# qasimyu/scssim

Hardware: AMD Instinct MI355X
Metric: paired-end read pairs/s (whole genreads job: MALBAC amplification + read allocation + read generation + FASTQ files, PE150 30x) (higher is better)
Workload: dtype u8/u32 (integer draws, byte sequences; fp64 only in the GC-weight draw and the allocation sums)

## Files before the change

scssim_amd/csrc/scs_device.h:

```cpp
#pragma once
#include <stdint.h>
#include <hip/hip_runtime.h>
#include "scs_common.h"
#include "scs_simuvars.h"

namespace scs {

struct DevFrags {
    const uint64_t* goff;
    const uint32_t* len;
    const int8_t*   strand;
    const uint32_t* primers;
    uint32_t n;
    uint64_t gidx_base;
    const uint8_t* has_n;
};

struct DevAmps {
    uint32_t* parent;
    uint32_t* sl;
    uint16_t* gc;
    uint16_t* primers;
    uint64_t* uid;
    uint64_t* errs;
};

struct DevGenomeIdx { const unsigned long long* gc_bits; const unsigned long long* n_bits; const uint64_t* gc_pref; const uint64_t* n_pref;
                      const ulonglong2* gc_pair; };

struct DevErrPool { uint32_t* data; uint32_t* head; uint32_t cap; };

struct View { int64_t base; int32_t dir; uint32_t comp; };

struct DevTables {
    int L, bins;
    uint32_t t_insert, t_delete, t_indel, t_ber;
    const uint32_t* gap_t; uint32_t t_kind;
    const uint32_t* subs1; const uint32_t* subs2;
    const uint32_t* qual;
    const uint4* ring1; const uint4* ring2;
    const uint4* ring1u; const uint4* ring2u;
    const uint32_t* qual_alias; int qual_k;
    const uint32_t* ins_t; int n_ins;
    const uint32_t* del_t; int n_del;
    const uint32_t* isize_t; int n_isize; int isize_min;
    const double* subs1_d; const double* subs2_d; const double* qual_d;
    const double* ins_d; const double* del_d; const double* isize_d;
    const double* gc_means; double gc_std;
};

struct AmplifyParams {
    RngKey key;
    uint32_t pass;
    uint32_t amp_min, amp_max;
    uint32_t t_ber;
};

struct PoissonParams {
    RngKey key; uint32_t call; double gamma;
    uint64_t total_primers;
    const uint64_t* totals;
    uint64_t nf, frag_len; const unsigned long long* dev;
    const unsigned long long* total_primers_dev;
};
enum { DS_HOLES = 20 };
enum { DS_SEMI_LEN = 4, DS_SEMIS_N = 5, DS_REPORTED_LEN = 6, DS_G_SEMIS_N = 8, DS_G_SEMI_LEN = 9, DS_G_PRIMERS = 10, DS_G_TOTALS = 11, DS_G_NF = 13, DS_G_FRAG_LEN = 14,
       DS_MIN_STOCK = 15 };
enum { SHARD_TAIL_WORDS = 16 };
struct AllocState { double total; unsigned long long sum_rn, sum_quota; };

#define ALLOC_CHUNK 1000u
enum { ALLOC_SLOTS = 40 };
struct AllocRange { uint32_t q0, c0, local0; };
struct AllocBChunk { uint32_t c, n, owner; };
struct AllocGSeg { unsigned long long go; uint32_t lo, n, owner, slot; };
struct AllocMySeg { unsigned long long go; uint32_t lo, n, order, pad; };
struct AllocPlan {
    unsigned long long total;
    uint32_t rank, n_interior, n_boundary, n_ranges, n_gseg;
    const AllocRange* rng; const AllocBChunk* bchunk; const AllocGSeg* gseg;
    AllocMySeg my_seg[ALLOC_SLOTS];
};
struct SegMap { uint32_t n; uint32_t lo[ALLOC_SLOTS], cnt[ALLOC_SLOTS]; unsigned long long go[ALLOC_SLOTS]; };

enum DevFlag : uint32_t { FLAG_ERRCAP = 1, FLAG_ERRPOOL = 2, FLAG_READSLOT = 4, FLAG_INTERNAL = 8, FLAG_KEYSPACE = 16, FLAG_TRUTH = 32, FLAG_DEPTH = 64, FLAG_AMP = 128, FLAG_SITE = 256, FLAG_SUPPORT = 512, FLAG_LIFT = 1024 };

struct PairRec {
    uint32_t amp, att, pos, isz;
    int64_t  base; uint32_t flags;
    int32_t  k1;
    uint64_t e1, e2, uid;
};

void launch_attach_frags(hipStream_t s, const uint8_t* g, DevFrags fr, const uint32_t* slot_off, uint32_t* slots,
                         uint32_t* slot_tmpl, uint32_t* valid, const unsigned long long* primer_cut, uint32_t* primer_delta,
                         unsigned long long* len_part, AmplifyParams p, uint32_t t_first, uint32_t t_end, int undo, const unsigned long long* t_from);
void launch_frag_len_sum(hipStream_t s, const unsigned long long* len_part, uint32_t nf, unsigned long long* len_sum);
void launch_poisson(hipStream_t s, DevFrags fr, DevAmps semis, uint32_t n_semis, PoissonParams p, uint32_t* budget_f, uint32_t* budget_s,
                    unsigned long long* sums, unsigned long long* part, uint32_t* flags);
void launch_alloc_bpack(hipStream_t s, const double* w, const AllocPlan& pl, double* send);
void launch_alloc_bgather(hipStream_t s, const double* w, const AllocPlan& pl, const double* gathered, double* brow, int* bmap);
void launch_alloc_chunk_sum(hipStream_t s, const double* w, const double* brow, const AllocPlan& pl, double* part);
void launch_tree_sum(hipStream_t s, const double* part, uint32_t nch, double* scratch, double* total);
void launch_alloc_norm(hipStream_t s, double* w, double* brow, const int* bmap, const AllocPlan& pl, const double* total, unsigned long long reads,
                       uint32_t* rn, double* tp, uint32_t* crn, unsigned long long* sum_rn);
void launch_alloc_quota(hipStream_t s, const double* tp, uint32_t nch, unsigned long long reads, const unsigned long long* sum_rn, unsigned long long* sum_quota,
                        uint32_t* quota, double* probs, double* scratch, RngKey key);
void launch_alloc_sample(hipStream_t s, const double* w, const double* brow, const int* bmap, const AllocPlan& pl, const double* tp, const uint32_t* quota, RngKey key, uint32_t* rn);
void launch_alloc_odd_scan(hipStream_t s, const uint32_t* rn, uint32_t ac, uint32_t* odd_before, void* temp, size_t temp_bytes);
void launch_alloc_odd_counts(hipStream_t s, const uint32_t* odd_before, const AllocPlan& pl, unsigned long long* table);
void launch_alloc_parity(hipStream_t s, uint32_t* rn, const uint32_t* odd_before, uint32_t ac, const AllocPlan& pl, const unsigned long long* table);
void launch_attach_semis(hipStream_t s, const uint8_t* g, DevFrags fr, DevAmps semis, uint32_t n_semis, DevErrPool spool,
                         const uint32_t* slot_off, uint32_t* slots, uint32_t* slot_tmpl, uint32_t* valid,
                         const unsigned long long* primer_cut, uint32_t* primer_delta, AmplifyParams p, uint32_t t_first, uint32_t t_end, int undo, const unsigned long long* t_from);
uint32_t attach_dense_waves(uint32_t n_slots);
void launch_attach_plan(hipStream_t s, const uint32_t* slot_off, uint32_t nt, uint32_t n_slots, uint32_t* item_tmpl, uint32_t* wave_first, uint32_t* valid);
void launch_attach_dense(hipStream_t s, const uint8_t* g, DevFrags fr, DevAmps semis, DevErrPool spool, const uint32_t* slot_off, uint32_t* slots, const uint32_t* item_tmpl,
                         const uint32_t* wave_first, uint32_t n_slots, uint32_t* valid, const unsigned long long* primer_cut, uint32_t* primer_delta, AmplifyParams p, int undo,
                         const unsigned long long* t_from);
void launch_stock_check(hipStream_t s, const int64_t* cnt, const uint32_t* taken, unsigned long long* cut, bool from_frag, unsigned long long* info);
void launch_stock_list(hipStream_t s, const int64_t* cnt, const uint32_t* taken, uint32_t* eidx, uint32_t* etype, uint32_t* estart, unsigned long long* info);
void launch_stock_collect(hipStream_t s, const uint8_t* g, DevFrags fr, DevAmps semis, DevErrPool spool, bool from_frag, const uint32_t* slot_off, const uint32_t* slots,
                          const uint32_t* valid, const uint32_t* eidx, unsigned long long* list, unsigned long long* info, uint32_t t_first, uint32_t t_end);
size_t stock_sort_temp_bytes(size_t n);
void launch_stock_sort(hipStream_t s, const unsigned long long* in, unsigned long long* out, size_t n, void* temp, size_t temp_bytes);
void launch_stock_pick(hipStream_t s, const int64_t* cnt, const uint32_t* etype, const uint32_t* estart, uint32_t ne, const unsigned long long* sorted, unsigned long long* cut,
                       bool from_frag, unsigned long long* info);
void launch_stock_apply(hipStream_t s, int64_t* cnt, uint32_t* gdelta, uint32_t* delta, unsigned long long* cut, uint32_t* flags);
void launch_errs_frags(hipStream_t s, const uint8_t* g, DevGenomeIdx gx, DevFrags fr, uint32_t n_slots, const uint32_t* slot_off, const uint32_t* slots,
                       const uint32_t* slot_tmpl, const uint32_t* valid_off, DevAmps out, uint32_t out_base, DevErrPool pool, uint32_t* flags,
                       const unsigned long long* binom, AmplifyParams p, int64_t* primer_cnt, uint32_t* primer_delta, unsigned long long* primer_cut, unsigned long long* sums,
                       unsigned long long* semis_n);
void launch_errs_semis(hipStream_t s, const uint8_t* g, DevGenomeIdx gx, DevFrags fr, DevAmps semis, uint32_t n_semis, DevErrPool spool, uint32_t n_slots,
                       const uint32_t* slot_off, const uint32_t* slots, const uint32_t* slot_tmpl, const uint32_t* valid_off,
                       DevAmps out, uint32_t out_base, DevErrPool pool, uint32_t* flags, const unsigned long long* binom, AmplifyParams p,
                       int64_t* primer_cnt, uint32_t* primer_delta, unsigned long long* primer_cut, unsigned long long* sums);
void launch_encode_bases(hipStream_t s, uint8_t* g, uint64_t n);
void launch_fa_gather_regular(hipStream_t s, const uint8_t* raw, uint8_t* dst, uint64_t n, uint32_t col0, uint32_t lb, uint32_t lw, uint32_t* ragged);
void launch_frag_has_n(hipStream_t s, const uint64_t* goff, const uint32_t* len, uint32_t nf, DevGenomeIdx gx, uint8_t* has_n);
size_t fasta_chunk_temp_bytes(uint32_t n);
void launch_fasta_chunk(hipStream_t s, const uint8_t* raw, uint32_t n, unsigned long long chunk_off, unsigned long long* st, uint8_t* kind, uint32_t* keep, uint32_t* pos,
                        uint8_t* out, unsigned long long* hdr, uint32_t hdr_cap, void* temp, size_t temp_bytes);
void launch_sv_build(hipStream_t s, const uint8_t* ref, const uint8_t* lit, const SvPiece* pieces, uint32_t np, const SvSubst* subs, uint32_t nsub, uint8_t* out, uint64_t total);
void launch_genome_bits(hipStream_t s, const uint8_t* g, uint64_t n, uint64_t nwords, unsigned long long* gc_bits, unsigned long long* n_bits,
                        uint32_t* gc_cnt, uint32_t* n_cnt, uint64_t* gc_pref, uint64_t* n_pref, void* temp, size_t temp_bytes, uint32_t* g2, ulonglong2* gc_pair);
void launch_amplify_init(hipStream_t s, int64_t* primer_cnt, unsigned long long* primer_cut, int64_t copies, uint32_t* primer_delta, uint32_t* primer_gdelta, uint32_t* flags, unsigned long long* sums,
                         unsigned long long nf_all, unsigned long long frag_len_all, unsigned long long total_primers, uint32_t* pool_head_a, uint32_t* pool_head_b);
void launch_primer_update(hipStream_t s, int64_t* primer_cnt, uint32_t* primer_delta, unsigned long long* primer_cut, unsigned long long* dsums, uint32_t* flags);
void launch_weights(hipStream_t s, DevAmps fulls, uint32_t n, DevTables tb, RngKey key, uint32_t frag_size, double* w);
void launch_plan_pairs(hipStream_t s, DevFrags fr, DevAmps semis, DevAmps fulls, uint32_t first, uint32_t n_fulls, uint32_t pair_lo, uint32_t pair_hi, const uint32_t* read_numbers,
                       const uint32_t* pair_off, SegMap gmap, DevTables tb, RngKey key, int paired, PairRec* pairs, unsigned long long* holes);
void launch_batch_bounds(hipStream_t s, const uint32_t* pair_off, uint32_t ac, unsigned long long batch, uint32_t nb, uint32_t* bounds);
void launch_parity_pair_offsets(hipStream_t s, uint32_t* rn, uint32_t ac, uint32_t* pair_cnt_off, void* temp, size_t temp_bytes);
void launch_pair_offsets(hipStream_t s, const uint32_t* rn, uint32_t ac, int paired, uint32_t* pair_cnt_off, void* temp, size_t temp_bytes);
struct ReadsSide {
    hipStream_t st[2] = {nullptr, nullptr}; hipEvent_t fork = nullptr, join[2] = {nullptr, nullptr}; void release();
    ReadsSide() = default; ReadsSide(const ReadsSide&) = delete; ReadsSide& operator=(const ReadsSide&) = delete; ~ReadsSide() { release(); }
};
size_t reads_lds_bytes(const DevTables& tb, bool uni = false);
struct BatchSet { uint32_t* ev_hdr; uint4* ev_dat; uint32_t* sizes[2]; uint64_t* off[2]; uint32_t *d1f[2], *d1p[2], *slist[2], *clist[2], *dlist[2]; };
struct BatchCounts { uint64_t bytes[2]; uint32_t n_general[2], n_one_event[2]; };
struct ReadsJob { const uint8_t* g; const uint32_t* g2; DevErrPool spool, fpool; DevTables tb; RngKey key; int paired; uint32_t slot; uint32_t* flags; ReadsSide* side; uint32_t amp_index_base = 0; };
void launch_reads(hipStream_t s, const ReadsJob& J, const PairRec* pairs, uint32_t np, const BatchSet& B, const BatchCounts& n, char* const out[2]);
void launch_read_lists(hipStream_t s, uint32_t np, int paired, const BatchSet& B, void* temp, size_t temp_bytes);
void phase_clock_report();
void launch_indels(hipStream_t s, const ReadsJob& J, const PairRec* pairs, uint32_t np, const BatchSet& B);
void launch_predict_windows(hipStream_t s, const uint8_t* windows, uint32_t n_reads, const uint64_t* uids, const uint32_t* atts,
                            const uint8_t* is_read1, DevTables tb, const DevTables* d_tb, RngKey key, uint32_t slot, char* slot_b, char* slot_q,
                            uint32_t* lens, uint32_t* flags);
void launch_text_checksum(hipStream_t s, const char* text, uint64_t nbytes, unsigned long long* out);
void launch_philox(hipStream_t s, const uint32_t* ctr, uint32_t n, RngKey key, uint32_t* out);
void launch_detlog(hipStream_t s, const double* x, uint32_t n, double* out);

#define MAIL_SEQ_SLOT 31
void launch_mail(hipStream_t s, const void* const* srcs, const int* widths, const int* dsts, int n, unsigned clear, unsigned long long* mail, unsigned long long seq);
void launch_shard_tail(hipStream_t s, uint32_t* primer_gdelta, const unsigned long long* dsums, const uint32_t* new_semis, int with_budgets);
void launch_primer_update_sharded(hipStream_t s, int64_t* primer_cnt, uint32_t* primer_gdelta, uint32_t* primer_delta, unsigned long long* primer_cut, unsigned long long* dsums, uint32_t* flags, int with_budgets);

hipError_t take_launch_error();

size_t scan_temp_bytes(size_t n);
size_t parity_scan_temp_bytes(size_t n);
void exclusive_scan_u32(hipStream_t s, const uint32_t* in, uint32_t* out, size_t n, void* temp, size_t temp_bytes);
void exclusive_scan_u32_pair(hipStream_t s, const uint32_t* in0, uint32_t* out0, size_t n0, const uint32_t* in1, uint32_t* out1, size_t n1, void* temp, size_t temp_bytes);
#define OFF_BITS 40
#define OFF_MASK ((1ull << OFF_BITS) - 1ull)
void exclusive_scan_sizes(hipStream_t s, const uint32_t* in, uint64_t* out, size_t n, void* temp, size_t temp_bytes);
void exclusive_scan_u32_to_u64(hipStream_t s, const uint32_t* in, uint64_t* out, size_t n, void* temp, size_t temp_bytes);

struct PlaceArgs {
    const PairRec* pairs; uint32_t np; int paired;
    const uint32_t* ev_hdr; const uint4* ev_dat;
    DevTables tb; RngKey key; uint32_t slot; uint32_t* flags;
};
struct TruthArgs : PlaceArgs {
    const uint64_t* off1; const uint64_t* off2; const char* fq1; const char* fq2;
    const uint8_t* g;
    const uint64_t* rec_off; const uint32_t* name_off; const char* names; uint32_t n_rec;
};
void launch_truth_size(hipStream_t s, const TruthArgs& a, uint32_t* sizes);
uint32_t truth_pairs_per_block(uint64_t fq_bytes, uint32_t np);
void launch_truth_emit(hipStream_t s, const TruthArgs& a, const uint64_t* offs, uint32_t pairs_per_block, char* out);
void launch_truth_bam_size(hipStream_t s, const TruthArgs& a, uint32_t* sizes);
uint32_t truth_bam_pairs_per_block(uint64_t fq_bytes, uint32_t np);
void launch_truth_bam_emit(hipStream_t s, const TruthArgs& a, const uint64_t* offs, uint32_t pairs_per_block, uint32_t lds, char* out);

struct DepthArgs : PlaceArgs {
    const uint64_t* rec_off; const uint64_t* bin_off; uint32_t n_rec;
    uint32_t bin_width, slots;
    unsigned long long* reads; unsigned long long* bases;
};
void launch_depth(hipStream_t s, const DepthArgs& a);

struct LiftSeg;
struct LiftArgs : PlaceArgs {
    const uint64_t* rec_off; uint32_t n_rec;
    const LiftSeg* segs; uint32_t n_seg;
    const uint64_t* ref_len; const uint64_t* ref_bin_off; uint32_t n_ref;
    uint32_t bin_width, slots; uint64_t n_bins;
    unsigned long long* reads; unsigned long long* bases;
};
void launch_depth_lift(hipStream_t s, const LiftArgs& a);
void launch_lift_copies(hipStream_t s, const LiftSeg* segs, uint32_t n_seg, const uint64_t* ref_len, const uint64_t* ref_bin_off, uint32_t n_ref, uint32_t bin_width,
                        uint64_t n_bins, unsigned long long* copies, uint32_t* flags);
void launch_lift_points(hipStream_t s, const LiftSeg* segs, uint32_t n_seg, const uint64_t* rec_off, uint32_t n_rec, const uint32_t* rec, const uint64_t* pos, uint64_t n,
                        uint32_t* ref_rec, uint64_t* ref_pos, uint32_t* kind, uint32_t* bad);

struct AmpArgs {
    DevFrags fr; DevAmps semis, fulls; const uint32_t* spool; const uint32_t* fpool;
    const uint8_t* g; const uint32_t* read_numbers;
    const uint64_t* rec_off; const uint32_t* name_off; const char* names; uint32_t n_rec;
    uint32_t first, n; uint32_t* flags;
};
#define AMP_LDS 16384u
void launch_amp_place(hipStream_t s, const AmpArgs& a, uint32_t* rec, uint64_t* start, uint32_t* len, int8_t* strand, uint32_t* n_edits);
void launch_amp_size(hipStream_t s, const AmpArgs& a, uint32_t* sizes);
void launch_amp_emit(hipStream_t s, const AmpArgs& a, const uint64_t* offs, uint32_t lds, char* out);

struct SiteRec;
struct SiteArgs {
    const uint64_t* keys; const uint32_t* reads; uint64_t n;
    const uint64_t* starts; const uint64_t* ps_start; const uint64_t* ends; const uint64_t* ps_end; uint64_t m;
    const uint8_t* g; const uint64_t* rec_off; const uint32_t* name_off; const char* names; uint32_t n_rec, min_reads; uint32_t* flags;
};
#define SITE_LDS 16384u
#define SITE_LDS_SLABS 1024u
void launch_site_count(hipStream_t s, const AmpArgs& a, uint64_t slab, uint32_t n_slabs, unsigned long long* cnt);
void launch_site_fill(hipStream_t s, const AmpArgs& a, uint64_t x0, uint64_t x1, unsigned long long* cur, uint64_t cap_e, uint64_t cap_a,
                      uint64_t* keys, uint32_t* kreads, uint64_t* starts, uint64_t* ends, uint32_t* areads);
void launch_site_check(hipStream_t s, const unsigned long long* cur, uint64_t n_e, uint64_t n_a, uint32_t* flags);
size_t site_sort_temp_bytes(size_t n);
void launch_site_sort(hipStream_t s, const uint64_t* keys_in, uint64_t* keys_out, const uint32_t* vals_in, uint32_t* vals_out, size_t n, unsigned end_bit, void* temp, size_t temp_bytes);
void launch_site_reduce(hipStream_t s, const SiteArgs& t, SiteRec* recs, uint32_t* sizes, uint32_t* keep);
void launch_site_emit(hipStream_t s, const SiteArgs& t, const SiteRec* recs, const uint64_t* offs, uint32_t lds, char* out, const uint32_t* site_pos = nullptr, const uint32_t* counts = nullptr);
void launch_site_compact(hipStream_t s, const SiteRec* recs, const uint32_t* keep, const uint32_t* pos, uint64_t n, SiteRec* out);

#define SUPPORT_MAX_POS ((1u << 29) - 1u)
#define SUPPORT_LDS_SLOTS 1024u
struct SupportArgs : PlaceArgs {
    const uint64_t* off1; const uint64_t* off2; const char* fq1; const char* fq2;
    const uint64_t* rec_off; uint32_t n_rec;
    const uint64_t* sp_pos; uint64_t n_pos;
    uint32_t* counts; uint32_t slots;
};
void launch_support(hipStream_t s, const SupportArgs& a);
void launch_support_heads(hipStream_t s, const SiteRec* sites, uint64_t n, const uint64_t* rec_off, uint32_t n_rec, uint32_t* head, uint32_t* flags);
void launch_support_scatter(hipStream_t s, const SiteRec* sites, uint64_t n, const uint64_t* rec_off, const uint32_t* head, const uint32_t* e, uint64_t* pos, uint32_t* site_pos);
void launch_support_size(hipStream_t s, const SiteArgs& t, const SiteRec* sites, const uint32_t* site_pos, const uint32_t* counts, uint32_t* sizes);

}
```

scssim_amd/csrc/scs_k_allocate.hip:

```cpp
#include <utility>
#include <type_traits>
#include "scs_device.h"
#include "scs_seams.h"

#include <algorithm>
#include <cstdlib>
#include <cstring>
#include <rocprim/rocprim.hpp>
#include "scs_kernels_common.h"

namespace scs {

struct GcDraw { double y, r2; bool in; };
__device__ __forceinline__ GcDraw gc_attempt(uint32_t wx, uint32_t wy) {
    const double x = 2.0 * (((double)wx + 0.5) / 4294967296.0) - 1.0;
    const double y = 2.0 * (((double)wy + 0.5) / 4294967296.0) - 1.0;
    const double r2 = x * x + y * y;
    return GcDraw{y, r2, !(r2 > 1.0 || r2 == 0.0)};
}
__device__ __forceinline__ double gc_value(double mean, double sd, double y, double r2) {
    const double mult = __dsqrt_rn(-2.0 * det_log(r2) / r2);
    return mean + sd * (y * mult);
}
constexpr int WEIGHTS_BLOCK = 1024;
__global__ __launch_bounds__(WEIGHTS_BLOCK) void k_weights(DevAmps fulls, uint32_t n, DevTables tb, RngKey key, uint32_t frag_size, double* __restrict__ w) {
    __shared__ uint32_t s_retry[WEIGHTS_BLOCK];
    __shared__ uint32_t s_n;
    if (threadIdx.x == 0) s_n = 0;
    __syncthreads();
    const uint32_t i = blockIdx.x * blockDim.x + threadIdx.x;
    const double scale = (double)(frag_size * frag_size), sd = tb.gc_std;
    if (i < n) {
        const uint32_t len = sl_len(fulls.sl[i]);
        const uint32_t gcp = 100u * fulls.gc[i] / len;
        if (gcp > 100) w[i] = 0.0 * (double)len / scale;
        else {
            const U4 d = draw4(key, ST_WEIGHT, 0, fulls.uid[i], 0);
            const GcDraw a0 = gc_attempt(d.w[0], d.w[1]), a1 = gc_attempt(d.w[2], d.w[3]);
            const bool any = a0.in || a1.in;
            double v = -1.0;
            if (any) v = gc_value(tb.gc_means[gcp], sd, a0.in ? a0.y : a1.y, a0.in ? a0.r2 : a1.r2);
            if (v < 0) s_retry[atomicAdd(&s_n, 1u)] = threadIdx.x | ((any && a0.in ? 1u : 2u) << 16);
            else w[i] = v * (double)len / scale;
        }
    }
    __syncthreads();
    const uint32_t nr = s_n;
    for (uint32_t k = threadIdx.x; k < nr; k += blockDim.x) {
        const uint32_t e = s_retry[k], j = blockIdx.x * blockDim.x + (e & 0xFFFFu);
        const uint32_t len = sl_len(fulls.sl[j]);
        const double mean = tb.gc_means[100u * fulls.gc[j] / len];
        const uint64_t uid = fulls.uid[j];
        uint32_t a = e >> 16;
        U4 d = draw4(key, ST_WEIGHT, 0, uid, a >> 1);
        double v;
        for (;; ++a) {
            if ((a & 1u) == 0 && a != (e >> 16)) d = draw4(key, ST_WEIGHT, 0, uid, a >> 1);
            const GcDraw t = (a & 1u) ? gc_attempt(d.w[2], d.w[3]) : gc_attempt(d.w[0], d.w[1]);
            if (!t.in) continue;
            v = gc_value(mean, sd, t.y, t.r2);
            if (v >= 0) break;
        }
        w[j] = v * (double)len / scale;
    }
}

__device__ __forceinline__ double shfl_xor_f64(double v, int d) {
    const long long b = __double_as_longlong(v);
    const int lo = __shfl_xor((int)b, d), hi = __shfl_xor((int)(b >> 32), d);
    return __longlong_as_double(((long long)hi << 32) | (unsigned int)lo);
}
__device__ __forceinline__ double shfl_up_f64(double v, int d) {
    const long long b = __double_as_longlong(v);
    const int lo = __shfl_up((int)b, d), hi = __shfl_up((int)(b >> 32), d);
    return __longlong_as_double(((long long)hi << 32) | (unsigned int)lo);
}
__device__ __forceinline__ double shfl_f64(double v, int src) {
    const long long b = __double_as_longlong(v);
    const int lo = __shfl((int)b, src), hi = __shfl((int)(b >> 32), src);
    return __longlong_as_double(((long long)hi << 32) | (unsigned int)lo);
}
__device__ __forceinline__ double wave_butterfly_f64(double acc) {
#pragma unroll
    for (int d = 32; d >= 1; d >>= 1) acc = acc + shfl_xor_f64(acc, d);
    return acc;
}
struct ChunkRef { uint32_t c, n, local0; int brow; bool owner; };
__device__ __forceinline__ ChunkRef chunk_ref(const AllocPlan& pl, uint32_t q) {
    ChunkRef r;
    if (q < pl.n_interior) {
        uint32_t k = 0;
        while (k + 1 < pl.n_ranges && q >= pl.rng[k + 1].q0) ++k;
        const AllocRange& g = pl.rng[k];
        r.c = g.c0 + (q - g.q0); r.local0 = g.local0 + (q - g.q0) * ALLOC_CHUNK; r.brow = -1; r.owner = true;
        const unsigned long long b = (unsigned long long)r.c * ALLOC_CHUNK;
        r.n = (uint32_t)min((unsigned long long)ALLOC_CHUNK, pl.total - b);
    } else {
        const uint32_t bi = q - pl.n_interior;
        r.c = pl.bchunk[bi].c; r.n = pl.bchunk[bi].n; r.local0 = 0; r.brow = (int)bi; r.owner = pl.bchunk[bi].owner != 0;
    }
    return r;
}
__global__ void __launch_bounds__(256) k_alloc_bpack(const double* __restrict__ w, AllocPlan pl, double* __restrict__ send) {
    const uint32_t slot = blockIdx.x / 2, half = blockIdx.x & 1u;
    const uint32_t n = pl.my_seg[slot].n, lo = pl.my_seg[slot].lo, m = min(n, ALLOC_CHUNK);
    for (uint32_t i = threadIdx.x; i < ALLOC_CHUNK; i += blockDim.x)
        send[((size_t)slot * 2 + half) * ALLOC_CHUNK + i] = i < m ? w[lo + (half ? n - m + i : i)] : 0.0;
}
__global__ void __launch_bounds__(256) k_alloc_bgather(const double* __restrict__ w, AllocPlan pl, const double* __restrict__ gathered,
                                                       double* __restrict__ brow, int* __restrict__ bmap) {
    const uint32_t bi = blockIdx.x;
    const unsigned long long g0 = (unsigned long long)pl.bchunk[bi].c * ALLOC_CHUNK;
    for (uint32_t e = threadIdx.x; e < ALLOC_CHUNK; e += blockDim.x) {
        double v = 0; int mp = -1;
        if (e < pl.bchunk[bi].n) {
            const unsigned long long gi = g0 + e;
            uint32_t lo = 0, hi = pl.n_gseg;
            while (hi - lo > 1) { const uint32_t mid = (lo + hi) >> 1; if (pl.gseg[mid].go <= gi) lo = mid; else hi = mid; }
            const AllocGSeg sg = pl.gseg[lo];
            const uint32_t j = (uint32_t)(gi - sg.go);
            if (sg.owner == pl.rank) { mp = (int)(sg.lo + j); v = w[sg.lo + j]; }
            else {
                const double* src = gathered + ((size_t)sg.owner * ALLOC_SLOTS + sg.slot) * 2 * ALLOC_CHUNK;
                v = j < ALLOC_CHUNK ? src[j] : src[ALLOC_CHUNK + (j - (sg.n - ALLOC_CHUNK))];
            }
        }
        brow[(size_t)bi * ALLOC_CHUNK + e] = v; bmap[(size_t)bi * ALLOC_CHUNK + e] = mp;
    }
}
__global__ void __launch_bounds__(256) k_alloc_chunk_sum(const double* __restrict__ w, const double* __restrict__ brow, AllocPlan pl,
                                                         double* __restrict__ part) {
    const uint32_t q = blockIdx.x * 4 + (threadIdx.x >> 6), lane = threadIdx.x & 63;
    if (q >= pl.n_interior + pl.n_boundary) return;
    const ChunkRef r = chunk_ref(pl, q);
    const double* __restrict__ v = r.brow < 0 ? w + r.local0 : brow + (size_t)r.brow * ALLOC_CHUNK;
    double acc = 0;
    for (uint32_t i = lane; i < r.n; i += WAVE) acc += v[i];
    acc = wave_butterfly_f64(acc);
    if (lane == 0 && r.owner) part[r.c] = acc;
}
__global__ void __launch_bounds__(256) k_tree1000(const double* __restrict__ in, uint32_t n, double* __restrict__ out) {
    const uint32_t gq = blockIdx.x * 4 + (threadIdx.x >> 6), lane = threadIdx.x & 63;
    const uint32_t b = gq * ALLOC_CHUNK;
    if (b >= n) return;
    const uint32_t m = min(ALLOC_CHUNK, n - b);
    double acc = 0;
    for (uint32_t i = lane; i < m; i += WAVE) acc += in[b + i];
    acc = wave_butterfly_f64(acc);
    if (lane == 0) out[gq] = acc;
}
__global__ void __launch_bounds__(256) k_alloc_norm(double* __restrict__ w, double* __restrict__ brow, const int* __restrict__ bmap, AllocPlan pl,
                                                    const double* __restrict__ total, unsigned long long reads, uint32_t* __restrict__ rn,
                                                    double* __restrict__ tp, uint32_t* __restrict__ crn) {
    const uint32_t q = blockIdx.x * 4 + (threadIdx.x >> 6), lane = threadIdx.x & 63;
    if (q >= pl.n_interior + pl.n_boundary) return;
    const ChunkRef r = chunk_ref(pl, q);
    double* __restrict__ v = r.brow < 0 ? w + r.local0 : brow + (size_t)r.brow * ALLOC_CHUNK;
    const int* __restrict__ mp = r.brow < 0 ? nullptr : bmap + (size_t)r.brow * ALLOC_CHUNK;
    const double den = 2.2204e-16 + *total;
    double acc = 0; uint32_t cs = 0;
    for (uint32_t i = lane; i < r.n; i += WAVE) {
        const double p = v[i] / den;
        v[i] = p; acc += p;
        const uint32_t c = (uint32_t)(p * (double)(long long)reads);
        if (mp) { const int li = mp[i]; if (li >= 0) { rn[li] = c; cs += c; } }
        else { rn[r.local0 + i] = c; cs += c; }
    }
    acc = wave_butterfly_f64(acc);
    cs = wave_sum(cs);
    if (lane == 0) { if (r.owner) tp[r.c] = acc; crn[q] = cs; }
}
__global__ void __launch_bounds__(1024) k_sum_u32(const uint32_t* __restrict__ v, uint32_t n, unsigned long long* __restrict__ dst, int add) {
    __shared__ unsigned long long s_p[16];
    unsigned long long acc = 0;
    for (uint32_t i = threadIdx.x; i < n; i += blockDim.x) acc += v[i];
    acc = wave_sum_u64(acc);
    if ((threadIdx.x & 63) == 0) s_p[threadIdx.x >> 6] = acc;
    __syncthreads();
    if (threadIdx.x == 0) { unsigned long long t = 0; for (int k = 0; k < 16; ++k) t += s_p[k]; *dst = add ? *dst + t : t; }
}
__global__ void __launch_bounds__(256) k_alloc_quota(const double* __restrict__ tp, uint32_t nch, unsigned long long reads, const unsigned long long* __restrict__ sum_rn,
                                                     uint32_t* __restrict__ quota) {
    const uint32_t c = blockIdx.x * blockDim.x + threadIdx.x;
    if (c >= nch) return;
    const unsigned long long nres = reads - *sum_rn;
    quota[c] = (uint32_t)(tp[c] * (double)nres);
}
__global__ void __launch_bounds__(64) k_scan1000(const double* __restrict__ in, uint32_t n, double* __restrict__ out, double* __restrict__ last) {
    const uint32_t g = blockIdx.x, b = g * ALLOC_CHUNK, m = min(ALLOC_CHUNK, n - b), lane = threadIdx.x;
    double carry = 0;
    for (uint32_t r = 0; r < m; r += WAVE) {
        double s = r + lane < m ? in[b + r + lane] : 0.0;
#pragma unroll
        for (int d = 1; d < WAVE; d <<= 1) { const double t = shfl_up_f64(s, d); if ((int)lane >= d) s = s + t; }
        if (r + lane < m) out[b + r + lane] = carry + s;
        carry = carry + shfl_f64(s, 63);
    }
    if (lane == 0 && last) last[g] = carry;
}
__global__ void __launch_bounds__(256) k_scan_fix(double* __restrict__ out, uint32_t n, const double* __restrict__ pre) {
    const uint32_t i = blockIdx.x * blockDim.x + threadIdx.x;
    if (i >= n || i < ALLOC_CHUNK) return;
    out[i] = pre[i / ALLOC_CHUNK - 1] + out[i];
}
__device__ __forceinline__ uint32_t first_le(const double* __restrict__ cdf, uint32_t n, double r) {
    uint32_t lo = 0, hi = n;
    while (lo < hi) { const uint32_t mid = (lo + hi) >> 1; if (r <= cdf[mid]) hi = mid; else lo = mid + 1; }
    return lo < n ? lo : n - 1;
}
__global__ void k_alloc_top_draws(const double* __restrict__ probs, uint32_t nch, unsigned long long reads, const unsigned long long* __restrict__ sum_rn,
                                  const unsigned long long* __restrict__ sum_quota, RngKey key, uint32_t* __restrict__ quota) {
    const uint32_t t = blockIdx.x * blockDim.x + threadIdx.x;
    const unsigned long long n = reads - *sum_rn - *sum_quota;
    if (t >= n) return;
    const U4 d = draw4(key, ST_ALLOC_TOP, 0, 0, t);
    const double r = 2.2204e-16 + (1 - 2.2204e-16) * ((double)d.w[0] / 4294967296.0);
    atomicAdd(&quota[first_le(probs, nch, r)], 1u);
}
__global__ void __launch_bounds__(256) k_alloc_sample(const double* __restrict__ w, const double* __restrict__ brow, const int* __restrict__ bmap, AllocPlan pl,
                                                      const double* __restrict__ tp, const uint32_t* __restrict__ quota, RngKey key, uint32_t* __restrict__ rn) {
    constexpr int ROUNDS = (ALLOC_CHUNK + WAVE - 1) / WAVE, WAVES = 4, MINE = ROUNDS / WAVES;
    static_assert(ROUNDS % WAVES == 0, "rounds of scan1000 divide among the waves");
    __shared__ double s_cdf[ALLOC_CHUNK];
    __shared__ uint32_t s_cnt[ALLOC_CHUNK];
    __shared__ double s_tot[ROUNDS];
    const uint32_t q = blockIdx.x, tid = threadIdx.x, lane = tid & 63u, wv = tid >> 6;
    const ChunkRef r = chunk_ref(pl, q);
    const uint32_t nq = quota[r.c];
    if (nq == 0) return;
    const double* __restrict__ v = r.brow < 0 ? w + r.local0 : brow + (size_t)r.brow * ALLOC_CHUNK;
    const double t = tp[r.c];
    double pv[MINE];
#pragma unroll
    for (int m = 0; m < MINE; ++m) { const uint32_t i = (uint32_t)((wv + WAVES * m) * WAVE) + lane; pv[m] = i < r.n ? v[i] : 0.0; }
#pragma unroll
    for (int m = 0; m < MINE; ++m) {
        const uint32_t k = wv + WAVES * m, i = k * WAVE + lane;
        double s = i < r.n ? pv[m] / t : 0.0;
#pragma unroll
        for (int d = 1; d < WAVE; d <<= 1) { const double u = shfl_up_f64(s, d); if ((int)lane >= d) s = s + u; }
        pv[m] = s;
        if (lane == 63) s_tot[k] = s;
    }
    __syncthreads();
#pragma unroll
    for (int m = 0; m < MINE; ++m) {
        const uint32_t k = wv + WAVES * m, i = k * WAVE + lane;
        double carry = 0;
        for (uint32_t z = 0; z < k; ++z) carry = carry + s_tot[z];
        if (i < r.n) { s_cdf[i] = carry + pv[m]; s_cnt[i] = 0; }
    }
    __syncthreads();
    for (uint32_t j = tid; 4u * j < nq; j += blockDim.x) {
        const U4 d = draw4(key, ST_ALLOC_CHUNK, 0, r.c, j);
        double x[4]; uint32_t lo[4], hi[4];
#pragma unroll
        for (int i = 0; i < 4; ++i) { x[i] = 2.2204e-16 + (1 - 2.2204e-16) * ((double)d.w[i] / 4294967296.0); lo[i] = 0; hi[i] = r.n; }
        for (uint32_t span = r.n; span; span >>= 1) {
#pragma unroll
            for (int i = 0; i < 4; ++i)
                if (lo[i] < hi[i]) { const uint32_t mid = (lo[i] + hi[i]) >> 1; if (x[i] <= s_cdf[mid]) hi[i] = mid; else lo[i] = mid + 1; }
        }
#pragma unroll
        for (int i = 0; i < 4; ++i) if (4u * j + (uint32_t)i < nq) atomicAdd(&s_cnt[lo[i] < r.n ? lo[i] : r.n - 1], 1u);
    }
    __syncthreads();
    for (uint32_t i = tid; i < r.n; i += blockDim.x) {
        const uint32_t c = s_cnt[i];
        if (!c) continue;
        if (r.brow < 0) rn[r.local0 + i] += c;
        else { const int li = bmap[(size_t)r.brow * ALLOC_CHUNK + i]; if (li >= 0) rn[li] += c; }
    }
}
__global__ void k_alloc_odd_counts(const uint32_t* __restrict__ odd_before, AllocPlan pl, unsigned long long* __restrict__ table) {
    const uint32_t slot = threadIdx.x;
    if (slot >= ALLOC_SLOTS) return;
    const uint32_t n = pl.my_seg[slot].n, lo = pl.my_seg[slot].lo;
    table[(size_t)pl.my_seg[slot].order] = n ? odd_before[lo + n] - odd_before[lo] : 0u;
}
__global__ void __launch_bounds__(256) k_alloc_parity(uint32_t* __restrict__ rn, const uint32_t* __restrict__ odd_before, uint32_t ac, AllocPlan pl,
                                                      const unsigned long long* __restrict__ table) {
    __shared__ unsigned long long s_base[ALLOC_SLOTS];
    if (threadIdx.x < ALLOC_SLOTS) {
        unsigned long long b = 0;
        if (table) { const uint32_t ord = pl.my_seg[threadIdx.x].order; for (uint32_t k = 0; k < ord; ++k) b += table[k]; }
        s_base[threadIdx.x] = b;
    }
    __syncthreads();
    const uint32_t i = blockIdx.x * blockDim.x + threadIdx.x;
    if (i >= ac) return;
    const uint32_t v = rn[i];
    if (!(v & 1u)) return;
    unsigned long long j = odd_before[i];
    if (table) {
        uint32_t k = 0;
        while (k + 1 < ALLOC_SLOTS && (pl.my_seg[k].n == 0 || i >= pl.my_seg[k].lo + pl.my_seg[k].n)) ++k;
        j = s_base[k] + (odd_before[i] - odd_before[pl.my_seg[k].lo]);
    }
    rn[i] = (j & 1ull) ? v - 1u : v + 1u;
}

struct OddBit { __host__ __device__ uint32_t operator()(uint32_t v) const { return v & 1u; } };
struct HalfUp { __host__ __device__ uint32_t operator()(uint32_t v) const { return (v + 1u) >> 1; } };

void launch_alloc_bpack(hipStream_t s, const double* w, const AllocPlan& pl, double* send) {
    hipLaunchKernelGGL(k_alloc_bpack, dim3(2 * ALLOC_SLOTS), dim3(256), 0, s, w, pl, send);
}
void launch_alloc_bgather(hipStream_t s, const double* w, const AllocPlan& pl, const double* gathered, double* brow, int* bmap) {
    if (pl.n_boundary) hipLaunchKernelGGL(k_alloc_bgather, dim3(pl.n_boundary), dim3(256), 0, s, w, pl, gathered, brow, bmap);
}
void launch_alloc_chunk_sum(hipStream_t s, const double* w, const double* brow, const AllocPlan& pl, double* part) {
    const uint32_t nq = pl.n_interior + pl.n_boundary;
    if (nq) hipLaunchKernelGGL(k_alloc_chunk_sum, dim3(cdiv(nq, 4)), dim3(256), 0, s, w, brow, pl, part);
}
void launch_tree_sum(hipStream_t s, const double* part, uint32_t nch, double* scratch, double* total) {
    if (nch == 0) { (void)hipMemsetAsync(total, 0, 8, s); return; }
    if (nch == 1) { (void)hipMemcpyAsync(total, part, 8, hipMemcpyDeviceToDevice, s); return; }
    const double* cur = part; uint32_t n = nch; double* nxt = scratch;
    while (n > 1) {
        const uint32_t ng = cdiv(n, ALLOC_CHUNK);
        double* dst = ng == 1 ? total : nxt;
        hipLaunchKernelGGL(k_tree1000, dim3(cdiv(ng, 4)), dim3(256), 0, s, cur, n, dst);
        cur = dst; nxt += ng; n = ng;
    }
}
void launch_alloc_norm(hipStream_t s, double* w, double* brow, const int* bmap, const AllocPlan& pl, const double* total, unsigned long long reads,
                       uint32_t* rn, double* tp, uint32_t* crn, unsigned long long* sum_rn) {
    const uint32_t nq = pl.n_interior + pl.n_boundary;
    if (nq) hipLaunchKernelGGL(k_alloc_norm, dim3(cdiv(nq, 4)), dim3(256), 0, s, w, brow, bmap, pl, total, reads, rn, tp, crn);
    hipLaunchKernelGGL(k_sum_u32, dim3(1), dim3(1024), 0, s, crn, nq, sum_rn, 0);
}
static void scan_all_dev(hipStream_t s, const double* in, uint32_t n, double* out, double* scratch) {
    const uint32_t ng = cdiv(n, ALLOC_CHUNK);
    double* last = scratch; double* pre = scratch + ng;
    hipLaunchKernelGGL(k_scan1000, dim3(ng), dim3(64), 0, s, in, n, out, ng > 1 ? last : (double*)nullptr);
    if (ng == 1) return;
    scan_all_dev(s, last, ng, pre, scratch + 2 * (size_t)ng);
    hipLaunchKernelGGL(k_scan_fix, dim3(cdiv(n, 256)), dim3(256), 0, s, out, n, pre);
}
void launch_alloc_quota(hipStream_t s, const double* tp, uint32_t nch, unsigned long long reads, const unsigned long long* sum_rn, unsigned long long* sum_quota,
                        uint32_t* quota, double* probs, double* scratch, RngKey key) {
    if (nch == 0) return;
    hipLaunchKernelGGL(k_alloc_quota, dim3(cdiv(nch, 256)), dim3(256), 0, s, tp, nch, reads, sum_rn, quota);
    hipLaunchKernelGGL(k_sum_u32, dim3(1), dim3(1024), 0, s, quota, nch, sum_quota, 0);
    scan_all_dev(s, tp, nch, probs, scratch);
    hipLaunchKernelGGL(k_alloc_top_draws, dim3(cdiv((uint64_t)nch + 1024, 256)), dim3(256), 0, s, probs, nch, reads, sum_rn, sum_quota, key, quota);
}
void launch_alloc_sample(hipStream_t s, const double* w, const double* brow, const int* bmap, const AllocPlan& pl, const double* tp, const uint32_t* quota, RngKey key, uint32_t* rn) {
    const uint32_t nq = pl.n_interior + pl.n_boundary;
    if (nq) hipLaunchKernelGGL(k_alloc_sample, dim3(nq), dim3(256), 0, s, w, brow, bmap, pl, tp, quota, key, rn);
}
void launch_alloc_odd_scan(hipStream_t s, const uint32_t* rn, uint32_t ac, uint32_t* odd_before, void* temp, size_t temp_bytes) {
    (void)rocprim::exclusive_scan(temp, temp_bytes, rocprim::make_transform_iterator(rn, OddBit()), odd_before, 0u, (size_t)ac + 1, rocprim::plus<uint32_t>(), s);
}
void launch_alloc_odd_counts(hipStream_t s, const uint32_t* odd_before, const AllocPlan& pl, unsigned long long* table) {
    hipLaunchKernelGGL(k_alloc_odd_counts, dim3(1), dim3(64), 0, s, odd_before, pl, table);
}
void launch_alloc_parity(hipStream_t s, uint32_t* rn, const uint32_t* odd_before, uint32_t ac, const AllocPlan& pl, const unsigned long long* table) {
    if (ac) hipLaunchKernelGGL(k_alloc_parity, dim3(cdiv(ac, 256)), dim3(256), 0, s, rn, odd_before, ac, pl, table);
}
void launch_weights(hipStream_t s, DevAmps fulls, uint32_t n, DevTables tb, RngKey key, uint32_t frag_size, double* w) {
    if (n == 0) return;
    hipLaunchKernelGGL(k_weights, dim3(cdiv(n, (uint32_t)WEIGHTS_BLOCK)), dim3(WEIGHTS_BLOCK), 0, s, fulls, n, tb, key, frag_size, w);
}
using ScanCfg = rocprim::scan_config<256, 16, rocprim::block_load_method::block_load_transpose, rocprim::block_store_method::block_store_transpose, rocprim::block_scan_algorithm::using_warp_scan>;
struct PackOddHalf { __host__ __device__ uint64_t operator()(uint32_t v) const { return ((uint64_t)(v & 1u) << 32) | (uint64_t)(v >> 1); } };
struct ParityOut {
    struct Ref {
        uint32_t* rn; uint32_t* pair_off; size_t ac, i;
        __device__ const Ref& operator=(uint64_t sum) const {
            const uint32_t odd = (uint32_t)(sum >> 32);
            pair_off[i] = (uint32_t)sum + ((odd + 1u) >> 1);
            if (i < ac) { const uint32_t v = rn[i]; if (v & 1u) rn[i] = (odd & 1u) ? v - 1u : v + 1u; }
            return *this;
        }
    };
    using iterator_category = std::random_access_iterator_tag; using value_type = uint64_t; using difference_type = std::ptrdiff_t;
    using pointer = void; using reference = Ref;
    uint32_t* rn; uint32_t* pair_off; size_t ac, at;
    __host__ __device__ Ref operator[](difference_type k) const { return Ref{rn, pair_off, ac, at + (size_t)k}; }
    __host__ __device__ Ref operator*() const { return Ref{rn, pair_off, ac, at}; }
    __host__ __device__ ParityOut operator+(difference_type k) const { return ParityOut{rn, pair_off, ac, at + (size_t)k}; }
    __host__ __device__ ParityOut operator-(difference_type k) const { return ParityOut{rn, pair_off, ac, at - (size_t)k}; }
    __host__ __device__ ParityOut& operator+=(difference_type k) { at += (size_t)k; return *this; }
    __host__ __device__ ParityOut& operator++() { ++at; return *this; }
    __host__ __device__ difference_type operator-(const ParityOut& o) const { return (difference_type)at - (difference_type)o.at; }
};
size_t parity_scan_temp_bytes(size_t n) {
    size_t c3 = 0;
    (void)rocprim::exclusive_scan<ScanCfg>(nullptr, c3, rocprim::make_transform_iterator((const uint32_t*)nullptr, PackOddHalf()), ParityOut{nullptr, nullptr, 0, 0},
                                  (uint64_t)0, n + 1, rocprim::plus<uint64_t>());
    return c3;
}
void launch_parity_pair_offsets(hipStream_t s, uint32_t* rn, uint32_t ac, uint32_t* pair_cnt_off, void* temp, size_t temp_bytes) {
    (void)rocprim::exclusive_scan<ScanCfg>(temp, temp_bytes, rocprim::make_transform_iterator((const uint32_t*)rn, PackOddHalf()), ParityOut{rn, pair_cnt_off, (size_t)ac, 0},
                                  (uint64_t)0, (size_t)ac + 1, rocprim::plus<uint64_t>(), s);
}
void launch_pair_offsets(hipStream_t s, const uint32_t* rn, uint32_t ac, int paired, uint32_t* pair_cnt_off, void* temp, size_t temp_bytes) {
    if (paired) (void)rocprim::exclusive_scan(temp, temp_bytes, rocprim::make_transform_iterator(rn, HalfUp()), pair_cnt_off, 0u, (size_t)ac + 1, rocprim::plus<uint32_t>(), s);
    else (void)rocprim::exclusive_scan(temp, temp_bytes, rn, pair_cnt_off, 0u, (size_t)ac + 1, rocprim::plus<uint32_t>(), s);
}
}
```

scssim_amd/csrc/scs_reads.cpp:

```cpp
#include "scs_sink.h"
#include <cerrno>

namespace scs {
void do_allocate(scs_ctx* c, uint64_t reads) {
    if (!c->amplified) throw ScsError(SCS_EINVAL, "scs_allocate_reads: call scs_amplify first");
    hipStream_t s = c->stream;
    if (reads == 0) {
        uint64_t ref_len = 0;
        for (auto& r : c->recs) { size_t p = r.name.rfind('_'); ref_len += (uint64_t)atoi(r.name.c_str() + (p == std::string::npos ? 0 : p + 1)); }
        ref_len /= 2;
        reads = (uint64_t)(ref_len * c->cfg.coverage / (long)c->prof.read_length);
    }
    if (c->cfg.verbose) fprintf(stderr, "\nNumber of reads to generate: %llu\n", (unsigned long long)reads);
    c->reads_requested = reads; c->st.reads_requested = reads;
    const uint32_t ac = c->fulls.n;
    double t0 = now_s();
    c->weights.reserve(std::max<size_t>((size_t)ac * 8, 16), s);
    c->read_numbers.reserve(((size_t)ac + 1) * 4, s); c->pair_off.reserve(((size_t)ac + 1) * 4, s);
    launch_weights(s, c->fulls.view(), ac, c->dtb, c->key, (uint32_t)c->cfg.frag_size, c->weights.as<double>());
    double* d_w = c->weights.as<double>(); uint32_t* d_rn = c->read_numbers.as<uint32_t>();

    const int R = c->cfg.shard_count, me = c->cfg.shard_rank; const bool multi = c->sharded();
    std::vector<uint64_t> segc((size_t)R * ALLOC_SLOTS, 0);
    for (auto& sg : c->full_segs) { if (sg.c < 0 || sg.c >= 5 || sg.p < 0 || sg.p >= 8) throw ScsError(SCS_EINVAL, "allocation: segment out of range"); segc[(size_t)me * ALLOC_SLOTS + sg.c * 8 + (7 - sg.p)] += sg.count; }
    if (multi) c->reduce(segc.data(), segc.size());
    std::vector<AllocGSeg> gseg; std::vector<uint32_t> loff(R, 0); uint64_t total = 0;
    AllocPlan pl{}; pl.rank = (uint32_t)me;
    for (int sl = 0; sl < ALLOC_SLOTS; ++sl) for (int r = 0; r < R; ++r) {
        const uint64_t n = segc[(size_t)r * ALLOC_SLOTS + sl];
        if (r == me) pl.my_seg[sl] = AllocMySeg{total, loff[r], (uint32_t)n, (uint32_t)(sl * R + r), 0};
        if (!n) continue;
        gseg.push_back(AllocGSeg{total, loff[r], (uint32_t)n, (uint32_t)r, (uint32_t)sl});
        loff[r] += (uint32_t)n; total += n;
    }
    if (loff[me] != ac) throw ScsError(SCS_EINVAL, "sharded allocation: segment bookkeeping mismatch");
    if (total > 0xFFFFFFF0ull) throw ScsError(SCS_EOVERFLOW, "more than 2^32 amplicons in the whole job");
    const uint32_t nch = (uint32_t)((total + ALLOC_CHUNK - 1) / ALLOC_CHUNK);
    std::vector<AllocRange> rng; std::vector<AllocBChunk> bch; uint32_t nq = 0;
    {
        auto owner_of = [&](uint64_t gi) { size_t lo = 0, hi = gseg.size(); while (hi - lo > 1) { const size_t mid = (lo + hi) / 2; if (gseg[mid].go <= gi) lo = mid; else hi = mid; } return gseg[lo].owner; };
        auto add_boundary = [&](uint32_t ch) { for (auto& b : bch) if (b.c == ch) return; bch.push_back(AllocBChunk{ch, (uint32_t)std::min<uint64_t>(ALLOC_CHUNK, total - (uint64_t)ch * ALLOC_CHUNK), owner_of((uint64_t)ch * ALLOC_CHUNK) == (uint32_t)me ? 1u : 0u}); };
        for (size_t k = 0; k < gseg.size();) {
            if (gseg[k].owner != (uint32_t)me) { ++k; continue; }
            uint64_t go = gseg[k].go, n = gseg[k].n; const uint32_t lo = gseg[k].lo; size_t j = k + 1;
            while (j < gseg.size() && gseg[j].owner == (uint32_t)me && gseg[j].go == go + n) { n += gseg[j].n; ++j; }
            k = j;
            const uint64_t cA = (go + ALLOC_CHUNK - 1) / ALLOC_CHUNK, cB = go + n == total ? nch : (go + n) / ALLOC_CHUNK;
            if (cA < cB) { rng.push_back(AllocRange{nq, (uint32_t)cA, (uint32_t)(lo + (cA * ALLOC_CHUNK - go))}); nq += (uint32_t)(cB - cA); }
            if (cA >= cB) { for (uint64_t ch = go / ALLOC_CHUNK; ch <= (go + n - 1) / ALLOC_CHUNK; ++ch) add_boundary((uint32_t)ch); }
            else {
                if (go % ALLOC_CHUNK) add_boundary((uint32_t)(go / ALLOC_CHUNK));
                if (cB * ALLOC_CHUNK < go + n) add_boundary((uint32_t)cB);
            }
        }
    }
    pl.total = total; pl.n_interior = nq; pl.n_boundary = (uint32_t)bch.size(); pl.n_ranges = (uint32_t)rng.size(); pl.n_gseg = (uint32_t)gseg.size();
    const uint32_t nwork = pl.n_interior + pl.n_boundary;
    {
        const size_t o_b = rng.size() * sizeof(AllocRange), o_g = o_b + bch.size() * sizeof(AllocBChunk), bytes = o_g + gseg.size() * sizeof(AllocGSeg);
        std::vector<uint8_t> blob(std::max<size_t>(bytes, 16));
        if (!rng.empty()) memcpy(blob.data(), rng.data(), o_b);
        if (!bch.empty()) memcpy(blob.data() + o_b, bch.data(), o_g - o_b);
        if (!gseg.empty()) memcpy(blob.data() + o_g, gseg.data(), bytes - o_g);
        c->a_plan.reserve(blob.size(), s);
        HIP_OK(hipMemcpyAsync(c->a_plan.p, blob.data(), blob.size(), hipMemcpyHostToDevice, s)); HIP_OK(hipStreamSynchronize(s));
        pl.rng = (const AllocRange*)c->a_plan.p; pl.bchunk = (const AllocBChunk*)((char*)c->a_plan.p + o_b); pl.gseg = (const AllocGSeg*)((char*)c->a_plan.p + o_g);
    }
    for (int sl = 0; sl < ALLOC_SLOTS; ++sl) c->seg_lo[sl] = pl.my_seg[sl].lo;
    c->seg_lo[ALLOC_SLOTS] = ac;
    c->gmap = SegMap{};
    if (multi) { uint32_t k = 0; for (int sl = 0; sl < ALLOC_SLOTS; ++sl) if (pl.my_seg[sl].n) { c->gmap.lo[k] = pl.my_seg[sl].lo; c->gmap.cnt[k] = pl.my_seg[sl].n; c->gmap.go[k] = pl.my_seg[sl].go; ++k; } c->gmap.n = k; }

    const size_t tree_scratch = (size_t)nch / ALLOC_CHUNK * 3 + 4096;
    c->a_part.reserve(((size_t)nch + 2) * 8, s); c->a_tp.reserve(((size_t)nch + 2) * 8, s); c->a_probs.reserve(((size_t)nch + 2) * 8, s);
    c->a_quota.reserve(((size_t)nch + 2) * 4, s); c->a_crn.reserve(((size_t)nwork + 2) * 4, s); c->a_scratch.reserve(tree_scratch * 8, s);
    c->a_brow.reserve(std::max<size_t>((size_t)pl.n_boundary * ALLOC_CHUNK * 8, 16), s); c->a_bmap.reserve(std::max<size_t>((size_t)pl.n_boundary * ALLOC_CHUNK * 4, 16), s);
    c->odd_before.reserve(((size_t)ac + 1) * 4, s); c->scan_tmp.reserve(scan_temp_bytes(ac), s);
    AllocState* st = (AllocState*)((char*)c->dsums.p + 128);
    double* d_part = c->a_part.as<double>(); double* d_tp = c->a_tp.as<double>();
    unsigned long long* d_sum_rn = (unsigned long long*)(d_tp + nch);
    if (R > 1) {
        const size_t per = (size_t)ALLOC_SLOTS * 2 * ALLOC_CHUNK * 8;
        c->a_send.reserve(per, s); c->a_gath.reserve(per * R, s);
        launch_alloc_bpack(s, d_w, pl, c->a_send.as<double>());
        c->gather_dev(c->a_send.p, c->a_gath.p, per);
    }
    launch_alloc_bgather(s, d_w, pl, c->a_gath.as<double>(), c->a_brow.as<double>(), c->a_bmap.as<int>());
    if (multi) HIP_OK(hipMemsetAsync(d_part, 0, (size_t)nch * 8, s));
    launch_alloc_chunk_sum(s, d_w, c->a_brow.as<double>(), pl, d_part);
    if (multi) c->reduce_dev(d_part, nch, 8);
    launch_tree_sum(s, d_part, nch, c->a_scratch.as<double>(), &st->total);
    if (multi) HIP_OK(hipMemsetAsync(d_tp, 0, ((size_t)nch + 1) * 8, s));
    launch_alloc_norm(s, d_w, c->a_brow.as<double>(), c->a_bmap.as<int>(), pl, &st->total, reads, d_rn, d_tp, c->a_crn.as<uint32_t>(), d_sum_rn);
    if (multi) c->reduce_dev(d_tp, (uint64_t)nch + 1, 8);
    launch_alloc_quota(s, d_tp, nch, reads, d_sum_rn, &st->sum_quota, c->a_quota.as<uint32_t>(), c->a_probs.as<double>(), c->a_scratch.as<double>(), c->key);
    launch_alloc_sample(s, d_w, c->a_brow.as<double>(), c->a_bmap.as<int>(), pl, d_tp, c->a_quota.as<uint32_t>(), c->key, d_rn);
    if (c->cfg.paired && !multi) launch_parity_pair_offsets(s, d_rn, ac, c->pair_off.as<uint32_t>(), c->scan_tmp.p, c->scan_tmp.cap);
    else if (c->cfg.paired) {
        launch_alloc_odd_scan(s, d_rn, ac, c->odd_before.as<uint32_t>(), c->scan_tmp.p, c->scan_tmp.cap);
        unsigned long long* table = nullptr;
        if (multi) {
            c->a_odd.reserve((size_t)R * ALLOC_SLOTS * 8, s); table = c->a_odd.as<unsigned long long>();
            HIP_OK(hipMemsetAsync(table, 0, (size_t)R * ALLOC_SLOTS * 8, s));
            launch_alloc_odd_counts(s, c->odd_before.as<uint32_t>(), pl, table);
            c->reduce_dev(table, (uint64_t)R * ALLOC_SLOTS, 8);
        }
        launch_alloc_parity(s, d_rn, c->odd_before.as<uint32_t>(), ac, pl, table);
    }
    if (!c->cfg.paired || multi) launch_pair_offsets(s, d_rn, ac, c->cfg.paired != 0, c->pair_off.as<uint32_t>(), c->scan_tmp.p, c->scan_tmp.cap);
    { Mail m; m.add(ac ? (const void*)(c->pair_off.as<uint32_t>() + ac) : nullptr, 4, 0); mail_post(c, m, true); }
    mail_wait(c);
    c->n_pairs_planned = (uint32_t)c->h_rb[0];
    c->st.t_stage[3] = 0; c->st.t_stage[4] = now_s() - t0;
    c->allocated = true;
}

BatchPlan plan_batches(uint64_t P, uint32_t L, bool to_sink, int writers, int regions, int batch_shift) {
    BatchPlan pl; regions = to_sink ? std::max(1, regions) : 1;
    uint64_t sink_batch = 1ull << 19;
    if (to_sink && writers > 4) {
        const uint64_t per_part = P / (2ull * (uint64_t)regions);
        sink_batch = 1ull << 18; while (sink_batch < (1ull << 21) && sink_batch * 2 <= per_part) sink_batch <<= 1;
        const uint64_t per_pair = 4ull * L + 64ull;
        while (sink_batch > (1ull << 18) && ((uint64_t)writers + 2ull) * sink_batch * per_pair > (24ull << 30)) sink_batch >>= 1;
    }
    pl.batch = std::min<uint64_t>(std::max<uint64_t>(P, 1), batch_shift ? (1ull << batch_shift) : to_sink ? sink_batch : (1ull << 23));
    const uint32_t nbatch = pl.nbatch = (uint32_t)((P + pl.batch - 1) / pl.batch);
    const int n_writers = to_sink ? std::max(1, std::min(writers, regions)) : 1;
    pl.order.reserve(nbatch); pl.region_of.reserve(nbatch);
    for (int g0 = 0; g0 < regions; g0 += n_writers) {
        const int g1 = std::min(regions, g0 + n_writers);
        std::vector<uint32_t> next((size_t)(g1 - g0)), end((size_t)(g1 - g0)); size_t left = 0;
        for (int r = g0; r < g1; ++r) { next[(size_t)(r - g0)] = (uint32_t)((uint64_t)nbatch * r / regions); end[(size_t)(r - g0)] = (uint32_t)((uint64_t)nbatch * (r + 1) / regions); left += end[(size_t)(r - g0)] - next[(size_t)(r - g0)]; }
        while (left) for (int r = g0; r < g1; ++r) if (next[(size_t)(r - g0)] < end[(size_t)(r - g0)]) { pl.order.push_back(next[(size_t)(r - g0)]++); pl.region_of.push_back((uint32_t)r); --left; }
    }
    return pl;
}

namespace {
struct Ship { char* p[3]; uint64_t n[3]; int dsl; uint32_t region; };
struct Batch { uint64_t it, p0; uint32_t bidx, np; int k, dsl; const PairRec* pr; const BatchSet* B; BatchCounts n; char* out[2]; char* t_text; uint64_t t_n; };
struct SegAt { size_t seg; uint32_t b; uint64_t o[2]; };
struct FdGuard { int fd = -1; ~FdGuard() { if (fd >= 0) ::close(fd); } };
struct PipeGuard { SinkPipe* p; ~PipeGuard() { if (p) (void)p->finish(); } };

struct Yield {
    scs_ctx* const c; const OutTarget& tg;
    const hipStream_t s = c->stream; hipStream_t ps = s; const int paired = c->cfg.paired != 0; const uint64_t P = c->n_pairs_planned; const uint32_t L = (uint32_t)c->prof.read_length, slot = ((L + 64 + 63) / 64) * 64;
    const bool to_sink = !tg.device && tg.sink, truth = !c->truth_path.empty(), bam = truth && c->truth_bam, bgzf = to_sink && tg.bgzf, depth = c->depth_width != 0, depth_ref = c->dref_width != 0, support = c->support_on; const std::string tname = bam ? "truth BAM" : "truth SAM";
    BatchPlan plan; std::vector<uint32_t> bounds; BatchSet bs[2]; ReadsJob job;
    uint64_t tot[2] = {0, 0}, sunk[2] = {0, 0}, truth_sum = 0, bi = 0;
    bool d2h_rec[2] = {false, false}, free_rec[2] = {false, false}; Ship pending{}; bool have_pending = false;
    FdGuard truth_fd;
    PipeGuard guard{nullptr}; TruthArgs ta{}; DepthArgs da{}; LiftArgs la{}; SupportArgs sa{};
    std::vector<uint64_t> bpair, bb[2]; std::vector<SegAt> seg_at;
    void truth_open() {
        truth_fd.fd = ::open(c->truth_path.c_str(), O_WRONLY | O_CREAT | O_TRUNC | O_CLOEXEC, 0644);
        if (truth_fd.fd < 0) throw ScsError(SCS_EIO, tname + ": can not open " + c->truth_path + ": " + strerror(errno));
        std::string hd = "@HD\tVN:1.6\tSO:unsorted\n"; const uint32_t nr = (uint32_t)c->recs.size();
        std::vector<uint64_t> roff(nr + 1, 0); std::vector<uint32_t> noff(nr + 1, 0); std::string names;
        for (uint32_t r = 0; r < nr; ++r) {
            hd += "@SQ\tSN:" + c->recs[r].name + "\tLN:" + std::to_string(c->rec_len[r]) + "\n";
            roff[r] = c->rec_off[r]; roff[r + 1] = c->rec_off[r] + c->rec_len[r];
            names += c->recs[r].name; noff[r + 1] = (uint32_t)names.size();
        }
        hd += "@PG\tID:scssim\tPN:scssim\n";
        if (bam) {
            std::string bh = "BAM\1";
            auto le32 = [&](uint32_t v) { for (int k = 0; k < 4; ++k) bh.push_back((char)(v >> (8 * k))); };
            le32((uint32_t)hd.size()); bh += hd; le32(nr);
            for (uint32_t r = 0; r < nr; ++r) { le32((uint32_t)c->recs[r].name.size() + 1u); bh += c->recs[r].name; bh.push_back('\0'); le32((uint32_t)c->rec_len[r]); }
            std::vector<uint8_t> z; bgzf_compress_host((const uint8_t*)bh.data(), bh.size(), BGZF_LDS_OUT, z);
            hd.assign((const char*)z.data(), z.size());
        }
        if (!SinkPipe::write_all(truth_fd.fd, hd.data(), hd.size())) throw ScsError(SCS_EIO, tname + ": writing " + c->truth_path + " failed");
        truth_sum = hd.size();
        const size_t o_name = (size_t)(nr + 1) * 8, o_text = o_name + (size_t)(nr + 1) * 4; std::vector<uint8_t> blob(o_text + names.size() + 16, 0);
        memcpy(blob.data(), roff.data(), o_name); memcpy(blob.data() + o_name, noff.data(), (size_t)(nr + 1) * 4); memcpy(blob.data() + o_text, names.data(), names.size());
        upload(c->t_recs, blob, s);
        c->t_sizes.reserve((plan.batch + 1) * 4, s); c->t_offs.reserve((plan.batch + 1) * 8, s); c->t_scan.reserve(scan_temp_bytes(plan.batch), s);
        c->h_t.reserve(64, hipHostMallocDefault); c->ev_t.ensure(hipEventDisableTiming | hipEventBlockingSync);
        HIP_OK(hipStreamSynchronize(s));
        const uint8_t* tb = c->t_recs.as<uint8_t>();
        ta.g = c->genome.as<uint8_t>(); ta.rec_off = (const uint64_t*)tb; ta.name_off = (const uint32_t*)(tb + o_name); ta.names = (const char*)(tb + o_text); ta.n_rec = nr;
        ta.paired = paired; ta.tb = c->dtb; ta.key = c->key; ta.slot = slot; ta.flags = c->flags.as<uint32_t>();
    }
    void depth_open() {
        static const uint32_t slots = seam_env("SCS_TEST_DEPTH_SLOTS") ? (uint32_t)atoi(seam_env("SCS_TEST_DEPTH_SLOTS")) : DEPTH_LDS_SLOTS;
        const uint32_t nr = (uint32_t)c->recs.size(); std::vector<uint64_t> tab(2 * ((size_t)nr + 1), 0), boff;
        const uint64_t nb = c->depth_bins = depth_ctx_layout(c, &boff);
        for (uint32_t r = 0; r < nr; ++r) { tab[r] = c->rec_off[r]; tab[r + 1] = c->rec_off[r] + c->rec_len[r]; }
        std::copy(boff.begin(), boff.end(), tab.begin() + nr + 1);
        upload(c->dp_tab, tab, s);
        c->dp_cnt.reserve(std::max<size_t>((size_t)nb * 16, 16), s); HIP_OK(hipMemsetAsync(c->dp_cnt.p, 0, std::max<size_t>((size_t)nb * 16, 16), s));
        HIP_OK(hipStreamSynchronize(s));
        da.rec_off = c->dp_tab.as<uint64_t>(); da.bin_off = da.rec_off + nr + 1; da.n_rec = nr; da.bin_width = c->depth_width; da.slots = slots;
        da.reads = c->dp_cnt.as<unsigned long long>(); da.bases = da.reads + nb;
        da.paired = paired; da.tb = c->dtb; da.key = c->key; da.slot = slot; da.flags = c->flags.as<uint32_t>();
    }
    void depth_ref_open() {
        static const uint32_t slots = seam_env("SCS_TEST_LIFT_SLOTS") ? (uint32_t)atoi(seam_env("SCS_TEST_LIFT_SLOTS")) : DEPTH_LDS_SLOTS;
        scs::depth_ref_open(c);
        const uint32_t nr = (uint32_t)c->recs.size(), nf = (uint32_t)c->lift.ref_lens.size(); const uint64_t nb = c->dref_bins;
        la.rec_off = c->dr_tab.as<uint64_t>(); la.n_rec = nr; la.ref_len = la.rec_off + nr + 1; la.ref_bin_off = la.ref_len + nf; la.n_ref = nf;
        la.segs = c->d_lift.as<LiftSeg>(); la.n_seg = (uint32_t)c->lift.segs.size(); la.bin_width = c->dref_width; la.slots = slots; la.n_bins = nb;
        la.reads = c->dr_cnt.as<unsigned long long>(); la.bases = la.reads + nb + 1;
        la.paired = paired; la.tb = c->dtb; la.key = c->key; la.slot = slot; la.flags = c->flags.as<uint32_t>();
    }
    void support_open() {
        static const uint32_t slots = seam_env("SCS_TEST_SUPPORT_SLOTS") ? (uint32_t)atoi(seam_env("SCS_TEST_SUPPORT_SLOTS")) : SUPPORT_LDS_SLOTS;
        scs::support_open(c);
        sa.rec_off = c->sp_tab.as<uint64_t>(); sa.n_rec = (uint32_t)c->recs.size(); sa.sp_pos = c->sp_pos.as<uint64_t>(); sa.n_pos = c->sp_n_pos;
        sa.counts = c->sp_cnt.as<uint32_t>(); sa.slots = slots;
        sa.paired = paired; sa.tb = c->dtb; sa.key = c->key; sa.slot = slot; sa.flags = c->flags.as<uint32_t>();
    }
    void setup() {
        bounds.assign(plan.nbatch + 1, 0);
        if (P) {
            c->d_bounds.reserve(((size_t)plan.nbatch + 1) * 4, s);
            launch_batch_bounds(s, c->pair_off.as<uint32_t>(), c->fulls.n, plan.batch, plan.nbatch, c->d_bounds.as<uint32_t>());
            HIP_OK(hipMemcpyAsync(bounds.data(), c->d_bounds.p, ((size_t)plan.nbatch + 1) * 4, hipMemcpyDeviceToHost, s)); HIP_OK(hipStreamSynchronize(s));
        }
        if (truth) truth_open();
        if (depth) depth_open();
        if (depth_ref) depth_ref_open();
        if (support) support_open();
        if (to_sink) {
            if (!c->pipe) c->pipe.reset(new SinkPipe);
            c->copy_stream.ensure(hipStreamNonBlocking); for (int k = 0; k < 2; ++k) { c->ev_made[k].ensure(hipEventDisableTiming); c->ev_d2h[k].ensure(hipEventDisableTiming); }
            c->pipe->truth_fd = truth_fd.fd; c->pipe->start(tg.sink, paired != 0, c->cfg.device); guard.p = c->pipe.get();
        }
        if (bgzf || bam) { c->h_z.reserve(64, hipHostMallocDefault); memset(c->h_z, 0, 64); for (int k = 0; k < 2; ++k) c->ev_z[k].ensure(hipEventDisableTiming | hipEventBlockingSync); }
        if ((bgzf || bam) && !c->z_crc.p) {
            std::vector<uint32_t> tabs(512); bgzf_host_tables(tabs.data(), tabs.data() + 256); upload(c->z_crc, tabs, s); HIP_OK(hipStreamSynchronize(s));
        }
        const uint64_t batch = plan.batch, nreads_b = paired ? 2 * batch : batch;
        c->ev_hdr.reserve(2 * nreads_b * 4, s); c->ev_dat.reserve(2 * nreads_b * 16, s);
        for (int m = 0; m < 2; ++m) c->sizes[m].reserve(2 * (batch + 1) * 4, s);
        for (int m = 0; m < 2; ++m) c->off[m].reserve(2 * (batch + 1) * 8, s);
        c->scan_tmp.reserve(scan_temp_bytes(batch), s);
        c->rl_cls.reserve(2 * (batch + 1) * 2 * 4, s); c->rl_pos.reserve(2 * (batch + 1) * 2 * 4, s); c->rl_lists.reserve(2 * batch * 6 * 4, s);
        for (int k = 0; k < 2; ++k) {
            BatchSet& B = bs[k]; B.ev_hdr = c->ev_hdr.as<uint32_t>() + k * nreads_b; B.ev_dat = c->ev_dat.as<uint4>() + k * nreads_b;
            for (int m = 0; m < 2; ++m) {
                B.sizes[m] = c->sizes[m].as<uint32_t>() + k * (batch + 1); B.off[m] = c->off[m].as<uint64_t>() + k * (batch + 1);
                B.d1f[m] = c->rl_cls.as<uint32_t>() + (k * 2 + m) * (batch + 1); B.d1p[m] = c->rl_pos.as<uint32_t>() + (k * 2 + m) * (batch + 1);
                B.slist[m] = c->rl_lists.as<uint32_t>() + (k * 6 + m) * batch; B.clist[m] = B.slist[m] + 2 * batch; B.dlist[m] = B.slist[m] + 4 * batch;
            }
        }
        job = ReadsJob{c->genome.as<uint8_t>(), c->genome2.as<uint32_t>() + 16, c->semis.pool_view(), c->fulls.pool_view(), c->dtb, c->key, paired, slot, c->flags.as<uint32_t>(), &c->reads_side};
        static const bool serial_pre = seam_env("SCS_READS_SERIAL") != nullptr;
        if (!serial_pre) {
            c->pre_stream.ensure(hipStreamNonBlocking); c->ev_plan.ensure(hipEventDisableTiming); for (int k = 0; k < 2; ++k) { c->ev_pre[k].ensure(hipEventDisableTiming); c->ev_free[k].ensure(hipEventDisableTiming); }
            ps = c->pre_stream; HIP_OK(hipEventRecord(c->ev_plan, s)); HIP_OK(hipStreamWaitEvent(ps, c->ev_plan, 0));
        }
        bb[0].assign(plan.nbatch, 0); bb[1].assign(plan.nbatch, 0);
        if (!tg.seg_off1) return;
        std::vector<uint32_t> v(ALLOC_SLOTS + 1, 0);
        for (int k = 0; k <= ALLOC_SLOTS; ++k) HIP_OK(hipMemcpyAsync(&v[k], c->pair_off.as<uint32_t>() + c->seg_lo[k], 4, hipMemcpyDeviceToHost, s));
        HIP_OK(hipStreamSynchronize(s));
        bpair.assign(v.begin(), v.end()); tg.seg_off1->assign(ALLOC_SLOTS + 1, 0); if (tg.seg_off2) tg.seg_off2->assign(ALLOC_SLOTS + 1, 0);
    }
    void prepass(uint64_t it) {
        hipStream_t s = ps;
        const int k = (int)(it & 1); const BatchSet& B = bs[k]; const uint64_t batch = plan.batch, p0 = (uint64_t)plan.order[it] * batch;
        if (ps != c->stream && free_rec[k]) HIP_OK(hipStreamWaitEvent(ps, c->ev_free[k], 0));
        const uint32_t np = (uint32_t)std::min<uint64_t>(batch, P - p0);
        const PairRec* pr = c->pairs.as<PairRec>() + p0;
        const uint32_t b = (uint32_t)(p0 / batch), a_lo = bounds[b], a_hi = std::min<uint32_t>(c->fulls.n, bounds[b + 1] + 1u);
        launch_plan_pairs(s, c->frags_view(), c->semis.view(), c->fulls.view(), a_lo, a_hi - a_lo, (uint32_t)p0, (uint32_t)(p0 + np), c->read_numbers.as<uint32_t>(), c->pair_off.as<uint32_t>(),
                          c->gmap, c->dtb, c->key, paired, c->pairs.as<PairRec>(), c->dsums.as<unsigned long long>() + DS_HOLES);
        c->tm[TM_INDELS].begin(s);
        launch_indels(s, job, pr, np, B);
        c->tm[TM_INDELS].end(s); c->tm[TM_INDELS].add_units(np);
        for (int m = 0; m < (paired ? 2 : 1); ++m) exclusive_scan_sizes(s, B.sizes[m], B.off[m], np, c->scan_tmp.p, c->scan_tmp.cap);
        launch_read_lists(s, np, paired, B, c->scan_tmp.p, c->scan_tmp.cap);
        Mail m; m.add(B.off[0] + np, 8, 0); m.add(paired ? (const void*)(B.off[1] + np) : nullptr, 8, 1);
        m.add(B.d1p[0] + np, 4, 2); m.add(paired ? (const void*)(B.d1p[1] + np) : nullptr, 4, 3); mail_post(c, m, true, s);
        if (ps != c->stream) HIP_OK(hipEventRecord(c->ev_pre[k], ps));
    }
    Batch decode(uint64_t it) const {
        Batch b{}; b.it = it; b.k = (int)(it & 1); b.bidx = plan.order[it]; b.p0 = (uint64_t)b.bidx * plan.batch; b.np = (uint32_t)std::min<uint64_t>(plan.batch, P - b.p0);
        b.pr = c->pairs.as<PairRec>() + b.p0; b.B = &bs[b.k]; b.dsl = (int)(bi & 1);
        for (int m = 0; m < 2; ++m) { b.n.bytes[m] = c->h_rb[m] & OFF_MASK; b.n.n_general[m] = (uint32_t)(c->h_rb[m] >> OFF_BITS); b.n.n_one_event[m] = (uint32_t)c->h_rb[2 + m]; }
        if (seam_env("SCS_DEBUG_CLASSES")) fprintf(stderr, "[classes] batch of %u pairs: general %u / %u, one-event %u / %u\n", b.np, b.n.n_general[0], b.n.n_general[1], b.n.n_one_event[0], b.n.n_one_event[1]);
        return b;
    }
    void index_batch(const Batch& b) {
        for (int m = 0; m < 2; ++m) bb[m][b.bidx] = b.n.bytes[m];
        for (size_t j = (size_t)(std::lower_bound(bpair.begin(), bpair.end(), b.p0) - bpair.begin()); j < bpair.size() && bpair[j] < b.p0 + b.np; ++j) {
            uint64_t ov[2] = {0, 0}; const uint64_t idx = bpair[j] - b.p0;
            for (int m = 0; m < (paired ? 2 : 1); ++m) HIP_OK(hipMemcpyAsync(&ov[m], b.B->off[m] + idx, 8, hipMemcpyDeviceToHost, s));
            HIP_OK(hipStreamSynchronize(s)); seg_at.push_back(SegAt{j, b.bidx, {ov[0] & OFF_MASK, ov[1] & OFF_MASK}});
        }
    }
    void reserve_slot(DevBuf* d, int nb, const uint64_t* need, const uint64_t* room, int dsl, bool stream_wait) {
        bool grows = false; for (int i = 0; i < nb; ++i) grows |= need[i] > d[i].cap;
        if (d2h_rec[dsl] && grows) HIP_OK(hipEventSynchronize(c->ev_d2h[dsl]));
        else if (d2h_rec[dsl] && stream_wait) HIP_OK(hipStreamWaitEvent(s, c->ev_d2h[dsl], 0));
        for (int i = 0; i < nb; ++i) d[i].reserve(room[i], s);
    }
    void base_pass(Batch& b) {
        if (tg.device) {
            if (tot[0] + b.n.bytes[0] > tg.cap1 || tot[1] + b.n.bytes[1] > tg.cap2) throw ScsError(SCS_EOVERFLOW, "scs_yield_reads_device: output buffer too small");
            b.out[0] = tg.d1 + tot[0]; b.out[1] = tg.d2 ? tg.d2 + tot[1] : nullptr;
        } else {
            DevBuf* d = c->out[b.dsl];
            const uint64_t want[2] = {std::max<uint64_t>(b.n.bytes[0] + b.n.bytes[0] / 16, 16), std::max<uint64_t>(b.n.bytes[1] + b.n.bytes[1] / 16, 16)};
            reserve_slot(d, 2, want, want, b.dsl, true);
            b.out[0] = d[0].as<char>(); b.out[1] = d[1].as<char>();
        }
        c->tm[TM_READS].begin(s);
        launch_reads(s, job, b.pr, b.np, *b.B, b.n, b.out);
        c->tm[TM_READS].end(s); c->tm[TM_READS].add_units(b.np);
        if (c->want_cks && !tg.device) for (int m = 0; m < 2; ++m) launch_text_checksum(s, b.out[m], m && !paired ? 0 : b.n.bytes[m], c->d_cks.as<unsigned long long>() + 2 * (size_t)b.bidx + m);
    }
    char* bgzf_in_place(int lane, const char* text, uint64_t n, int dsl, const char* too_large) {
        if (bgzf_bound(n) > 0xFFFFFFF0ull) throw ScsError(SCS_EOVERFLOW, too_large);
        scs_ctx::BgzfLane& z = c->z[lane]; DevBuf& zo = z.out[dsl]; const uint32_t nblk = bgzf_blocks(n); const uint64_t zb = bgzf_bound(n);
        z.plan.reserve(std::max<size_t>((size_t)nblk * BGZF_PLAN_BYTES, 16), s); z.sizes.reserve(((size_t)nblk + 2) * 4, s); z.offs.reserve(((size_t)nblk + 2) * 4, s);
        reserve_slot(&zo, 1, &zb, &zb, dsl, false);
        launch_bgzf_plan(s, text, n, z.plan.as<uint8_t>(), z.sizes.as<uint32_t>());
        exclusive_scan_u32(s, z.sizes.as<uint32_t>(), z.offs.as<uint32_t>(), nblk, nullptr, 0);
        launch_bgzf_emit(s, text, n, z.plan.as<uint8_t>(), z.sizes.as<uint32_t>(), z.offs.as<uint32_t>(), c->z_crc.as<uint32_t>(), c->z_crc.as<uint32_t>() + 256, zo.as<char>(), 0);
        HIP_OK(hipMemcpyAsync(c->h_z + (dsl * 3 + lane), z.offs.as<uint32_t>() + nblk, 4, hipMemcpyDeviceToHost, s));
        return zo.as<char>();
    }
    void truth_batch(Batch& b) {
        static const uint32_t bam_lds = seam_env("SCS_TEST_TRUTH_LDS") ? (uint32_t)atoi(seam_env("SCS_TEST_TRUTH_LDS")) : 0u;
        const uint32_t np = b.np; const uint64_t fq_bytes = b.n.bytes[0] + b.n.bytes[1];
        ta.pairs = b.pr; ta.np = np; ta.ev_hdr = b.B->ev_hdr; ta.ev_dat = b.B->ev_dat; ta.off1 = b.B->off[0]; ta.off2 = b.B->off[1]; ta.fq1 = b.out[0]; ta.fq2 = b.out[1];
        c->tm[TM_TRUTH].begin(s);
        if (bam) launch_truth_bam_size(s, ta, c->t_sizes.as<uint32_t>()); else launch_truth_size(s, ta, c->t_sizes.as<uint32_t>());
        exclusive_scan_u32_to_u64(s, c->t_sizes.as<uint32_t>(), c->t_offs.as<uint64_t>(), np, c->t_scan.p, c->t_scan.cap);
        HIP_OK(hipMemcpyAsync(c->h_t, c->t_offs.as<uint64_t>() + np, 8, hipMemcpyDeviceToHost, s)); HIP_OK(hipEventRecord(c->ev_t, s));
        c->tm[TM_TRUTH].end(s);
        HIP_OK(hipEventSynchronize(c->ev_t));
        { const hipError_t le = take_launch_error(); if (le != hipSuccess) throw ScsError(SCS_EDEVICE, std::string("truth sizing pass failed: ") + hipGetErrorString(le)); }
        DevBuf& to = c->t_out[b.dsl]; const uint64_t t_n = *c->h_t, need = std::max<uint64_t>(t_n, 16), room = std::max<uint64_t>(t_n + t_n / 16, 16);
        reserve_slot(&to, 1, &need, &room, b.dsl, false);
        c->tm[TM_TRUTH].begin(s);
        if (!bam) {
            launch_truth_emit(s, ta, c->t_offs.as<uint64_t>(), truth_pairs_per_block(fq_bytes, np), to.as<char>());
            b.t_text = to.as<char>(); b.t_n = t_n; truth_sum += t_n;
        } else if (t_n) {
            launch_truth_bam_emit(s, ta, c->t_offs.as<uint64_t>(), truth_bam_pairs_per_block(fq_bytes, np), bam_lds, to.as<char>());
            b.t_text = bgzf_in_place(2, to.as<char>(), t_n, b.dsl, "truth BAM: a batch's records exceed 4 GB");
            if (!bgzf) HIP_OK(hipEventRecord(c->ev_z[b.dsl], s));
        }
        c->tm[TM_TRUTH].end(s); c->tm[TM_TRUTH].add_units(np);
    }
    void depth_batch(const Batch& b) {
        da.pairs = b.pr; da.np = b.np; da.ev_hdr = b.B->ev_hdr; da.ev_dat = b.B->ev_dat;
        c->tm[TM_DEPTH].begin(s);
        launch_depth(s, da);
        c->tm[TM_DEPTH].end(s); c->tm[TM_DEPTH].add_units(b.np);
    }
    void depth_ref_batch(const Batch& b) {
        la.pairs = b.pr; la.np = b.np; la.ev_hdr = b.B->ev_hdr; la.ev_dat = b.B->ev_dat;
        c->tm_depth_ref.begin(s);
        launch_depth_lift(s, la);
        c->tm_depth_ref.end(s); c->tm_depth_ref.add_units(b.np);
    }
    void support_batch(const Batch& b) {
        sa.pairs = b.pr; sa.np = b.np; sa.ev_hdr = b.B->ev_hdr; sa.ev_dat = b.B->ev_dat; sa.off1 = b.B->off[0]; sa.off2 = b.B->off[1]; sa.fq1 = b.out[0]; sa.fq2 = b.out[1];
        c->tm_support.begin(s);
        launch_support(s, sa);
        c->tm_support.end(s); c->tm_support.add_units(b.np);
    }
    void ship(Ship sh) {
        if (bgzf || (bam && sh.p[2])) HIP_OK(hipEventSynchronize(c->ev_z[sh.dsl]));
        if (bgzf) { sh.n[0] = c->h_z[sh.dsl * 3]; sh.n[1] = c->h_z[sh.dsl * 3 + 1]; }
        if (bam && sh.p[2]) { sh.n[2] = c->h_z[sh.dsl * 3 + 2]; truth_sum += sh.n[2]; }
        const int hs = c->pipe->acquire(sh.n[0], sh.n[1], sh.n[2]);
        if (hs < 0) throw ScsError(SCS_EIO, "sink aborted");
        SinkPipe::Slot& H = c->pipe->slots[(size_t)hs];
        HIP_OK(hipStreamWaitEvent(c->copy_stream, c->ev_made[sh.dsl], 0));
        for (int f = 0; f < 3; ++f) if (sh.n[f]) HIP_OK(hipMemcpyAsync(H.h[f], sh.p[f], sh.n[f], hipMemcpyDeviceToHost, c->copy_stream));
        HIP_OK(hipEventRecord(H.ev, c->copy_stream));
        HIP_OK(hipEventRecord(c->ev_d2h[sh.dsl], c->copy_stream)); d2h_rec[sh.dsl] = true;
        c->pipe->submit((int)sh.region, hs, sh.n[0], sh.n[1], sh.n[2]);
        sunk[0] += sh.n[0]; sunk[1] += sh.n[1];
    }
    void sink_batch(const Batch& b) {
        Ship sh{{b.out[0], b.out[1], b.t_text}, {tg.discard ? 0 : b.n.bytes[0], tg.discard ? 0 : b.n.bytes[1], b.t_n}, b.dsl, plan.region_of[b.it]};
        if (bgzf) {
            for (int m = 0; m < (paired ? 2 : 1); ++m) sh.p[m] = bgzf_in_place(m, b.out[m], b.n.bytes[m], b.dsl, "BGZF: a batch's text exceeds 4 GB");
            if (!paired) { c->h_z[b.dsl * 3 + 1] = 0; sh.p[1] = nullptr; }
            HIP_OK(hipEventRecord(c->ev_z[b.dsl], s));
        }
        HIP_OK(hipEventRecord(c->ev_made[b.dsl], s));
        if (bgzf) { if (have_pending) ship(pending); pending = sh; have_pending = true; } else ship(sh);
        ++bi;
    }
    void finish(uint64_t* n1_out, uint64_t* n2_out, uint64_t* pairs_out) {
        std::vector<uint64_t>* so[2] = {tg.seg_off1, tg.seg_off2};
        for (int m = 0; m < 2 && tg.seg_off1; ++m) {
            if (!so[m]) continue;
            std::vector<uint64_t> pre(plan.nbatch + 1, 0);
            for (uint32_t b = 0; b < plan.nbatch; ++b) pre[b + 1] = pre[b] + bb[m][b];
            for (size_t j = 0; j < bpair.size(); ++j) (*so[m])[j] = tot[m];
            for (const SegAt& a : seg_at) (*so[m])[a.seg] = pre[a.b] + a.o[m];
        }
        { Mail m; m.add(c->flags.p, 4, 30); m.add(c->dsums.as<unsigned long long>() + DS_HOLES, 8, 2); mail_post(c, m, true); }
        HIP_OK(hipStreamSynchronize(s));
        if (to_sink) { HIP_OK(hipStreamSynchronize(c->copy_stream)); guard.p = nullptr; const bool ok = c->pipe->finish(); c->pipe->truth_fd = -1; if (!ok) throw ScsError(SCS_EIO, truth ? "sink aborted (or the " + tname + " could not be written)" : std::string("sink aborted")); }
        if (bam) {
            static const unsigned char eof[28] = {0x1f, 0x8b, 0x08, 0x04, 0, 0, 0, 0, 0, 0xff, 0x06, 0, 0x42, 0x43, 0x02, 0, 0x1b, 0, 0x03, 0, 0, 0, 0, 0, 0, 0, 0, 0};
            if (!SinkPipe::write_all(truth_fd.fd, (const char*)eof, 28)) throw ScsError(SCS_EIO, "truth BAM: writing " + c->truth_path + " failed");
            truth_sum += 28;
        }
        if (truth) { const int fd = truth_fd.fd; truth_fd.fd = -1; if (::close(fd) != 0) throw ScsError(SCS_EIO, tname + ": closing " + c->truth_path + " failed"); c->truth_bytes = truth_sum; }
        mail_wait(c); flags_eval(c);
        if (c->want_cks && !tg.device && plan.nbatch) { c->cks.assign((size_t)plan.nbatch * 2, 0); HIP_OK(hipMemcpyAsync(c->cks.data(), c->d_cks.p, (size_t)plan.nbatch * 16, hipMemcpyDeviceToHost, s)); HIP_OK(hipStreamSynchronize(s)); }
        const uint64_t pairs_written = P - c->h_rb[2];
        c->tm[TM_READS].collect(); c->tm[TM_INDELS].collect(); c->tm[TM_TRUTH].collect(); c->tm[TM_DEPTH].collect(); c->tm_support.collect(); c->tm_depth_ref.collect();
        c->depth_valid = depth; c->support_valid = support; c->dref_valid = depth_ref;
        c->st.pairs_written = pairs_written; c->st.reads_written = paired ? 2 * pairs_written : pairs_written;
        for (int m = 0; m < 2; ++m) { c->st.fastq_bytes[m] = tot[m]; c->st.sink_bytes[m] = to_sink ? sunk[m] : 0; }
        const uint64_t per_pair_tmpl = paired ? (uint64_t)(c->cfg.isize + 1) : (uint64_t)L;
        c->st.algorithmic_bytes = 1526ull * (c->st.semi_amplicons + c->st.full_amplicons) + pairs_written * per_pair_tmpl + tot[0] + tot[1];
        if (n1_out) *n1_out = tot[0]; if (n2_out) *n2_out = tot[1]; if (pairs_out) *pairs_out = pairs_written;
        if (seam_env("SCS_PHASE_CLOCK")) phase_clock_report();
        if (c->cfg.verbose) fprintf(stderr, "\nReads generation done!\n");
    }
};
}

void do_yield(scs_ctx* c, const OutTarget& tg, uint64_t* n1_out, uint64_t* n2_out, uint64_t* pairs_out) {
    if (!c->allocated) throw ScsError(SCS_EINVAL, "scs_yield_reads: call scs_allocate_reads first");
    Yield y{c, tg}; const hipStream_t s = y.s; const uint64_t P = y.P;
    if (c->cfg.verbose) fprintf(stderr, "\n*****Producing reads*****\n");
    c->timing_gate = (c->yield_calls++ % c->timing_every) == 0;
    c->tm[TM_READS].reset(); c->tm[TM_INDELS].reset(); c->tm[TM_TRUTH].reset(); c->tm[TM_DEPTH].reset(); c->tm_support.reset(); c->tm_depth_ref.reset();
    c->depth_valid = false; c->support_valid = false; c->dref_valid = false;
    if (c->depth_width) (void)depth_ctx_layout(c, nullptr);
    if (c->dref_width) { depth_ref_check(c); (void)depth_ref_layout(c, nullptr); }
    if (y.paired && P > 0 && c->prof.isize_t.empty()) throw ScsError(SCS_EIO, "Error: unrecognized parameter name \"insertSize\"");
    c->pairs.reserve(std::max<size_t>(P * sizeof(PairRec), 16), s); HIP_OK(hipMemsetAsync(c->dsums.as<unsigned long long>() + DS_HOLES, 0, 8, s));
    if (y.truth) { truth_check(c, tg.device, y.to_sink ? tg.sink->writers : 1); if (!y.to_sink) throw ScsError(SCS_EINVAL, y.tname + ": the reads must go to a sink"); }
    if (y.bam) {
        for (size_t r = 0; r < c->rec_len.size(); ++r)
            if (c->rec_len[r] >= (1ull << 29)) throw ScsError(SCS_EINVAL, "truth BAM (scs_set_truth_bam): record " + c->recs[r].name + " has 2^29 bases or more (the BAM bin scheme ends there); the truth SAM (scs_set_truth_sam) has no such limit");
        if ((y.paired ? 2 * P : P) > 0x7FFFFFFFull) throw ScsError(SCS_EINVAL, "truth BAM (scs_set_truth_bam): more than 2^31 - 1 records");
    }
    if (y.support) {
        support_check(c);
        if ((y.paired ? 2 * P : P) >> 32) throw ScsError(SCS_EINVAL, "site support (scs_set_site_support): 2^32 reads or more are planned (the counters are 32 bits wide)");
    }
    static const int batch_shift = seam_env("SCS_TEST_BATCH_SHIFT") ? atoi(seam_env("SCS_TEST_BATCH_SHIFT")) : 0;
    y.plan = plan_batches(P, y.L, y.to_sink, y.to_sink ? tg.sink->writers : 1, y.to_sink ? tg.sink->regions : 1, batch_shift);
    y.setup();
    c->cks.clear(); if (c->want_cks && !tg.device) c->d_cks.reserve(std::max<size_t>((size_t)y.plan.nbatch * 16, 16), s);
    if (P) y.prepass(0);
    for (uint64_t it = 0; it < y.plan.nbatch; ++it) {
        mail_wait(c);
        Batch b = y.decode(it);
        if (y.ps != s) HIP_OK(hipStreamWaitEvent(s, c->ev_pre[b.k], 0));
        if (it + 1 < y.plan.nbatch) y.prepass(it + 1);
        y.index_batch(b);
        y.base_pass(b);
        if (y.truth) y.truth_batch(b);
        if (y.depth) y.depth_batch(b);
        if (y.depth_ref) y.depth_ref_batch(b);
        if (y.support) y.support_batch(b);
        if (y.ps != s) { HIP_OK(hipEventRecord(c->ev_free[b.k], s)); y.free_rec[b.k] = true; }
        { const hipError_t le = take_launch_error(); if (le != hipSuccess) throw ScsError(SCS_EDEVICE, std::string("k_reads launch failed: ") + hipGetErrorString(le)); }
        if (y.to_sink) y.sink_batch(b);
        for (int m = 0; m < 2; ++m) y.tot[m] += b.n.bytes[m];
    }
    if (y.have_pending) y.ship(y.pending);
    y.finish(n1_out, n2_out, pairs_out);
}

void truth_check(scs_ctx* c, bool device, int writers) {
    if (c->truth_path.empty()) return;
    const std::string fn = c->truth_bam ? "scs_set_truth_bam" : "scs_set_truth_sam", what = (c->truth_bam ? "truth BAM (" : "truth SAM (") + fn + ")";
    if (device) throw ScsError(SCS_EINVAL, what + ": not available with scs_yield_reads_device; turn it off with " + fn + "(ctx, NULL)");
    if (c->cfg.shard_count > 1 || c->sliced) throw ScsError(SCS_EINVAL, what + ": not available for a sharded job (shard_count > 1)");
    if (writers > 1) throw ScsError(SCS_EINVAL, what + ": needs writers <= 1 (part files are made out of record order)");
}

void depth_check(scs_ctx* c) {
    depth_ref_check(c);
    if (!c->depth_width) return;
    if (c->cfg.shard_count > 1 || c->sliced) throw ScsError(SCS_EINVAL, "depth track (scs_set_depth): not available for a sharded job (shard_count > 1); turn it off with scs_set_depth(ctx, 0)");
}
uint64_t depth_ctx_layout(const scs_ctx* c, std::vector<uint64_t>* bin_off) {
    const size_t nr = c->rec_len.size(); uint64_t nb = 0; uint32_t min_w = 0;
    if (bin_off) bin_off->assign(nr + 1, 0);
    if (depth_layout(c->rec_len.data(), nr, c->depth_width, bin_off ? bin_off->data() : nullptr, &nb, &min_w)) return nb;
    throw ScsError(SCS_EINVAL, "depth track (scs_set_depth): bins of " + std::to_string(c->depth_width) + " bases give more than 2^27 bins for the staged genome; " +
                   (min_w ? "the smallest bin width it admits is " + std::to_string(min_w) : std::string("no bin width below 2^32 is enough")));
}

}
```

Measured before the change: 54.68 million.

## Fuse GC weight draw with per-chunk sums and drop in-place normalisation

The weight kernel now runs one wave per allocation chunk (plus gap pieces that fall outside interior chunks). It draws GC weights, handles rejection retries with a wave-level work queue, and writes each interior chunk's partial sum directly, so the separate chunk-sum pass only covers boundary chunks. The normalisation kernel no longer writes probabilities back into the weight array; the sampler divides by the total itself. This removes a full read-and-write pass over the weights, but the retry loop changes from block-wide to per-wave and adds host-side gap bookkeeping.

```diff
diff --git a/scssim_amd/csrc/scs_device.h b/scssim_amd/csrc/scs_device.h
--- a/scssim_amd/csrc/scs_device.h
+++ b/scssim_amd/csrc/scs_device.h
@@ -74,11 +74,12 @@
 struct AllocRange { uint32_t q0, c0, local0; };
 struct AllocBChunk { uint32_t c, n, owner; };
 struct AllocGSeg { unsigned long long go; uint32_t lo, n, owner, slot; };
+struct AllocGap { uint32_t lo, n; };
 struct AllocMySeg { unsigned long long go; uint32_t lo, n, order, pad; };
 struct AllocPlan {
     unsigned long long total;
-    uint32_t rank, n_interior, n_boundary, n_ranges, n_gseg;
-    const AllocRange* rng; const AllocBChunk* bchunk; const AllocGSeg* gseg;
+    uint32_t rank, n_interior, n_boundary, n_ranges, n_gseg, n_gap;
+    const AllocRange* rng; const AllocBChunk* bchunk; const AllocGSeg* gseg; const AllocGap* gap;
     AllocMySeg my_seg[ALLOC_SLOTS];
 };
 struct SegMap { uint32_t n; uint32_t lo[ALLOC_SLOTS], cnt[ALLOC_SLOTS]; unsigned long long go[ALLOC_SLOTS]; };
@@ -100,13 +101,13 @@
                     unsigned long long* sums, unsigned long long* part, uint32_t* flags);
 void launch_alloc_bpack(hipStream_t s, const double* w, const AllocPlan& pl, double* send);
 void launch_alloc_bgather(hipStream_t s, const double* w, const AllocPlan& pl, const double* gathered, double* brow, int* bmap);
-void launch_alloc_chunk_sum(hipStream_t s, const double* w, const double* brow, const AllocPlan& pl, double* part);
+void launch_alloc_chunk_sum(hipStream_t s, const double* brow, const AllocPlan& pl, double* part);
 void launch_tree_sum(hipStream_t s, const double* part, uint32_t nch, double* scratch, double* total);
-void launch_alloc_norm(hipStream_t s, double* w, double* brow, const int* bmap, const AllocPlan& pl, const double* total, unsigned long long reads,
+void launch_alloc_norm(hipStream_t s, const double* w, const double* brow, const int* bmap, const AllocPlan& pl, const double* total, unsigned long long reads,
                        uint32_t* rn, double* tp, uint32_t* crn, unsigned long long* sum_rn);
 void launch_alloc_quota(hipStream_t s, const double* tp, uint32_t nch, unsigned long long reads, const unsigned long long* sum_rn, unsigned long long* sum_quota,
                         uint32_t* quota, double* probs, double* scratch, RngKey key);
-void launch_alloc_sample(hipStream_t s, const double* w, const double* brow, const int* bmap, const AllocPlan& pl, const double* tp, const uint32_t* quota, RngKey key, uint32_t* rn);
+void launch_alloc_sample(hipStream_t s, const double* w, const double* brow, const int* bmap, const AllocPlan& pl, const double* total, const double* tp, const uint32_t* quota, RngKey key, uint32_t* rn);
 void launch_alloc_odd_scan(hipStream_t s, const uint32_t* rn, uint32_t ac, uint32_t* odd_before, void* temp, size_t temp_bytes);
 void launch_alloc_odd_counts(hipStream_t s, const uint32_t* odd_before, const AllocPlan& pl, unsigned long long* table);
 void launch_alloc_parity(hipStream_t s, uint32_t* rn, const uint32_t* odd_before, uint32_t ac, const AllocPlan& pl, const unsigned long long* table);
@@ -147,7 +148,7 @@
 void launch_amplify_init(hipStream_t s, int64_t* primer_cnt, unsigned long long* primer_cut, int64_t copies, uint32_t* primer_delta, uint32_t* primer_gdelta, uint32_t* flags, unsigned long long* sums,
                          unsigned long long nf_all, unsigned long long frag_len_all, unsigned long long total_primers, uint32_t* pool_head_a, uint32_t* pool_head_b);
 void launch_primer_update(hipStream_t s, int64_t* primer_cnt, uint32_t* primer_delta, unsigned long long* primer_cut, unsigned long long* dsums, uint32_t* flags);
-void launch_weights(hipStream_t s, DevAmps fulls, uint32_t n, DevTables tb, RngKey key, uint32_t frag_size, double* w);
+void launch_weights(hipStream_t s, DevAmps fulls, const AllocPlan& pl, DevTables tb, RngKey key, uint32_t frag_size, double* w, double* part);
 void launch_plan_pairs(hipStream_t s, DevFrags fr, DevAmps semis, DevAmps fulls, uint32_t first, uint32_t n_fulls, uint32_t pair_lo, uint32_t pair_hi, const uint32_t* read_numbers,
                        const uint32_t* pair_off, SegMap gmap, DevTables tb, RngKey key, int paired, PairRec* pairs, unsigned long long* holes);
 void launch_batch_bounds(hipStream_t s, const uint32_t* pair_off, uint32_t ac, unsigned long long batch, uint32_t nb, uint32_t* bounds);
diff --git a/scssim_amd/csrc/scs_k_allocate.hip b/scssim_amd/csrc/scs_k_allocate.hip
--- a/scssim_amd/csrc/scs_k_allocate.hip
+++ b/scssim_amd/csrc/scs_k_allocate.hip
@@ -10,60 +10,6 @@
 #include "scs_kernels_common.h"
 
 namespace scs {
-
-struct GcDraw { double y, r2; bool in; };
-__device__ __forceinline__ GcDraw gc_attempt(uint32_t wx, uint32_t wy) {
-    const double x = 2.0 * (((double)wx + 0.5) / 4294967296.0) - 1.0;
-    const double y = 2.0 * (((double)wy + 0.5) / 4294967296.0) - 1.0;
-    const double r2 = x * x + y * y;
-    return GcDraw{y, r2, !(r2 > 1.0 || r2 == 0.0)};
-}
-__device__ __forceinline__ double gc_value(double mean, double sd, double y, double r2) {
-    const double mult = __dsqrt_rn(-2.0 * det_log(r2) / r2);
-    return mean + sd * (y * mult);
-}
-constexpr int WEIGHTS_BLOCK = 1024;
-__global__ __launch_bounds__(WEIGHTS_BLOCK) void k_weights(DevAmps fulls, uint32_t n, DevTables tb, RngKey key, uint32_t frag_size, double* __restrict__ w) {
-    __shared__ uint32_t s_retry[WEIGHTS_BLOCK];
-    __shared__ uint32_t s_n;
-    if (threadIdx.x == 0) s_n = 0;
-    __syncthreads();
-    const uint32_t i = blockIdx.x * blockDim.x + threadIdx.x;
-    const double scale = (double)(frag_size * frag_size), sd = tb.gc_std;
-    if (i < n) {
-        const uint32_t len = sl_len(fulls.sl[i]);
-        const uint32_t gcp = 100u * fulls.gc[i] / len;
-        if (gcp > 100) w[i] = 0.0 * (double)len / scale;
-        else {
-            const U4 d = draw4(key, ST_WEIGHT, 0, fulls.uid[i], 0);
-            const GcDraw a0 = gc_attempt(d.w[0], d.w[1]), a1 = gc_attempt(d.w[2], d.w[3]);
-            const bool any = a0.in || a1.in;
-            double v = -1.0;
-            if (any) v = gc_value(tb.gc_means[gcp], sd, a0.in ? a0.y : a1.y, a0.in ? a0.r2 : a1.r2);
-            if (v < 0) s_retry[atomicAdd(&s_n, 1u)] = threadIdx.x | ((any && a0.in ? 1u : 2u) << 16);
-            else w[i] = v * (double)len / scale;
-        }
-    }
-    __syncthreads();
-    const uint32_t nr = s_n;
-    for (uint32_t k = threadIdx.x; k < nr; k += blockDim.x) {
-        const uint32_t e = s_retry[k], j = blockIdx.x * blockDim.x + (e & 0xFFFFu);
-        const uint32_t len = sl_len(fulls.sl[j]);
-        const double mean = tb.gc_means[100u * fulls.gc[j] / len];
-        const uint64_t uid = fulls.uid[j];
-        uint32_t a = e >> 16;
-        U4 d = draw4(key, ST_WEIGHT, 0, uid, a >> 1);
-        double v;
-        for (;; ++a) {
-            if ((a & 1u) == 0 && a != (e >> 16)) d = draw4(key, ST_WEIGHT, 0, uid, a >> 1);
-            const GcDraw t = (a & 1u) ? gc_attempt(d.w[2], d.w[3]) : gc_attempt(d.w[0], d.w[1]);
-            if (!t.in) continue;
-            v = gc_value(mean, sd, t.y, t.r2);
-            if (v >= 0) break;
-        }
-        w[j] = v * (double)len / scale;
-    }
-}
 
 __device__ __forceinline__ double shfl_xor_f64(double v, int d) {
     const long long b = __double_as_longlong(v);
@@ -101,6 +47,89 @@
     }
     return r;
 }
+struct GcDraw { double y, r2; bool in; };
+__device__ __forceinline__ GcDraw gc_attempt(uint32_t wx, uint32_t wy) {
+    const double x = 2.0 * (((double)wx + 0.5) / 4294967296.0) - 1.0;
+    const double y = 2.0 * (((double)wy + 0.5) / 4294967296.0) - 1.0;
+    const double r2 = x * x + y * y;
+    return GcDraw{y, r2, !(r2 > 1.0 || r2 == 0.0)};
+}
+__device__ __forceinline__ double gc_value(double mean, double sd, double y, double r2) {
+    const double mult = __dsqrt_rn(-2.0 * det_log(r2) / r2);
+    return mean + sd * (y * mult);
+}
+__device__ __forceinline__ void wave_lds_sync() { __builtin_amdgcn_fence(__ATOMIC_ACQ_REL, "wavefront"); __builtin_amdgcn_wave_barrier(); }
+constexpr int WEIGHTS_WAVES = 4;
+__global__ __launch_bounds__(WEIGHTS_WAVES * WAVE) void k_weights(DevAmps fulls, AllocPlan pl, DevTables tb, RngKey key, uint32_t frag_size, double* __restrict__ w,
+                                                                  double* __restrict__ part) {
+    __shared__ double s_val[WEIGHTS_WAVES][ALLOC_CHUNK];
+    __shared__ uint16_t s_queue[WEIGHTS_WAVES][ALLOC_CHUNK];
+    const uint32_t wv = threadIdx.x >> 6, lane = threadIdx.x & 63, q = blockIdx.x * WEIGHTS_WAVES + wv;
+    if (q >= pl.n_interior + pl.n_gap) return;
+    uint32_t base, n, c = 0; const bool chunk = q < pl.n_interior;
+    if (chunk) { const ChunkRef r = chunk_ref(pl, q); base = r.local0; n = r.n; c = r.c; }
+    else { base = pl.gap[q - pl.n_interior].lo; n = pl.gap[q - pl.n_interior].n; }
+    double* __restrict__ val = s_val[wv]; uint16_t* __restrict__ queue = s_queue[wv];
+    const double scale = (double)(frag_size * frag_size), sd = tb.gc_std;
+    const unsigned long long below = (1ull << lane) - 1ull;
+    uint32_t nq = 0;
+    uint32_t sl = 0, gc = 0; uint64_t uid = 0;
+    if (lane < n) { sl = fulls.sl[base + lane]; gc = fulls.gc[base + lane]; uid = fulls.uid[base + lane]; }
+    for (uint32_t i = lane; i - lane < n; i += WAVE) {
+        const uint32_t sl0 = sl, gc0 = gc; const uint64_t uid0 = uid;
+        if (i + WAVE < n) { sl = fulls.sl[base + i + WAVE]; gc = fulls.gc[base + i + WAVE]; uid = fulls.uid[base + i + WAVE]; }
+        uint32_t first = 0;
+        if (i < n) {
+            const uint32_t len = sl_len(sl0);
+            const uint32_t gcp = 100u * gc0 / len;
+            double v = 0.0;
+            if (gcp <= 100) {
+                const U4 d = draw4(key, ST_WEIGHT, 0, uid0, 0);
+                const GcDraw a0 = gc_attempt(d.w[0], d.w[1]), a1 = gc_attempt(d.w[2], d.w[3]);
+                const bool any = a0.in || a1.in;
+                v = -1.0;
+                if (any) v = gc_value(tb.gc_means[gcp], sd, a0.in ? a0.y : a1.y, a0.in ? a0.r2 : a1.r2);
+                if (v < 0) first = any && a0.in ? 1u : 2u;
+            }
+            if (!first) { v = v * (double)len / scale; w[base + i] = v; val[i] = v; }
+        }
+        const unsigned long long b = __ballot(first != 0);
+        if (first) queue[nq + (uint32_t)__popcll(b & below)] = (uint16_t)(i | (first << 10));
+        nq += (uint32_t)__popcll(b);
+    }
+    wave_lds_sync();
+    uint32_t next = min(nq, (uint32_t)WAVE), k = lane, a = 0, i = 0, len = 0; double mean = 0; U4 d{}; bool fresh = false;
+    bool have = k < nq;
+    auto take = [&]() {
+        const uint32_t e = queue[k];
+        i = e & 1023u; a = e >> 10; fresh = true;
+        len = sl_len(fulls.sl[base + i]); mean = tb.gc_means[100u * fulls.gc[base + i] / len]; uid = fulls.uid[base + i];
+    };
+    if (have) take();
+    while (__ballot(have)) {
+        bool done = false;
+        if (have) {
+            if (fresh || (a & 1u) == 0) d = draw4(key, ST_WEIGHT, 0, uid, a >> 1);
+            fresh = false;
+            const GcDraw t = (a & 1u) ? gc_attempt(d.w[2], d.w[3]) : gc_attempt(d.w[0], d.w[1]);
+            ++a;
+            if (t.in) {
+                double v = gc_value(mean, sd, t.y, t.r2);
+                if (v >= 0) { done = true; v = v * (double)len / scale; w[base + i] = v; val[i] = v; }
+            }
+        }
+        const unsigned long long b = __ballot(done);
+        if (done) { k = next + (uint32_t)__popcll(b & below); have = k < nq; if (have) take(); }
+        next += (uint32_t)__popcll(b);
+    }
+    if (!chunk) return;
+    wave_lds_sync();
+    double acc = 0;
+    for (uint32_t j = lane; j < n; j += WAVE) acc += val[j];
+    acc = wave_butterfly_f64(acc);
+    if (lane == 0) part[c] = acc;
+}
+
 __global__ void __launch_bounds__(256) k_alloc_bpack(const double* __restrict__ w, AllocPlan pl, double* __restrict__ send) {
     const uint32_t slot = blockIdx.x / 2, half = blockIdx.x & 1u;
     const uint32_t n = pl.my_seg[slot].n, lo = pl.my_seg[slot].lo, m = min(n, ALLOC_CHUNK);
@@ -128,12 +157,11 @@
         brow[(size_t)bi * ALLOC_CHUNK + e] = v; bmap[(size_t)bi * ALLOC_CHUNK + e] = mp;
     }
 }
-__global__ void __launch_bounds__(256) k_alloc_chunk_sum(const double* __restrict__ w, const double* __restrict__ brow, AllocPlan pl,
-                                                         double* __restrict__ part) {
-    const uint32_t q = blockIdx.x * 4 + (threadIdx.x >> 6), lane = threadIdx.x & 63;
+__global__ void __launch_bounds__(256) k_alloc_chunk_sum(const double* __restrict__ brow, AllocPlan pl, double* __restrict__ part) {
+    const uint32_t q = pl.n_interior + blockIdx.x * 4 + (threadIdx.x >> 6), lane = threadIdx.x & 63;
     if (q >= pl.n_interior + pl.n_boundary) return;
     const ChunkRef r = chunk_ref(pl, q);
-    const double* __restrict__ v = r.brow < 0 ? w + r.local0 : brow + (size_t)r.brow * ALLOC_CHUNK;
+    const double* __restrict__ v = brow + (size_t)r.brow * ALLOC_CHUNK;
     double acc = 0;
     for (uint32_t i = lane; i < r.n; i += WAVE) acc += v[i];
     acc = wave_butterfly_f64(acc);
@@ -149,19 +177,19 @@
     acc = wave_butterfly_f64(acc);
     if (lane == 0) out[gq] = acc;
 }
-__global__ void __launch_bounds__(256) k_alloc_norm(double* __restrict__ w, double* __restrict__ brow, const int* __restrict__ bmap, AllocPlan pl,
+__global__ void __launch_bounds__(256) k_alloc_norm(const double* __restrict__ w, const double* __restrict__ brow, const int* __restrict__ bmap, AllocPlan pl,
                                                     const double* __restrict__ total, unsigned long long reads, uint32_t* __restrict__ rn,
                                                     double* __restrict__ tp, uint32_t* __restrict__ crn) {
     const uint32_t q = blockIdx.x * 4 + (threadIdx.x >> 6), lane = threadIdx.x & 63;
     if (q >= pl.n_interior + pl.n_boundary) return;
     const ChunkRef r = chunk_ref(pl, q);
-    double* __restrict__ v = r.brow < 0 ? w + r.local0 : brow + (size_t)r.brow * ALLOC_CHUNK;
+    const double* __restrict__ v = r.brow < 0 ? w + r.local0 : brow + (size_t)r.brow * ALLOC_CHUNK;
     const int* __restrict__ mp = r.brow < 0 ? nullptr : bmap + (size_t)r.brow * ALLOC_CHUNK;
     const double den = 2.2204e-16 + *total;
     double acc = 0; uint32_t cs = 0;
     for (uint32_t i = lane; i < r.n; i += WAVE) {
         const double p = v[i] / den;
-        v[i] = p; acc += p;
+        acc += p;
         const uint32_t c = (uint32_t)(p * (double)(long long)reads);
         if (mp) { const int li = mp[i]; if (li >= 0) { rn[li] = c; cs += c; } }
         else { rn[r.local0 + i] = c; cs += c; }
@@ -218,7 +246,8 @@
     atomicAdd(&quota[first_le(probs, nch, r)], 1u);
 }
 __global__ void __launch_bounds__(256) k_alloc_sample(const double* __restrict__ w, const double* __restrict__ brow, const int* __restrict__ bmap, AllocPlan pl,
-                                                      const double* __restrict__ tp, const uint32_t* __restrict__ quota, RngKey key, uint32_t* __restrict__ rn) {
+                                                      const double* __restrict__ total, const double* __restrict__ tp, const uint32_t* __restrict__ quota, RngKey key,
+                                                      uint32_t* __restrict__ rn) {
     constexpr int ROUNDS = (ALLOC_CHUNK + WAVE - 1) / WAVE, WAVES = 4, MINE = ROUNDS / WAVES;
     static_assert(ROUNDS % WAVES == 0, "rounds of scan1000 divide among the waves");
     __shared__ double s_cdf[ALLOC_CHUNK];
@@ -229,14 +258,14 @@
     const uint32_t nq = quota[r.c];
     if (nq == 0) return;
     const double* __restrict__ v = r.brow < 0 ? w + r.local0 : brow + (size_t)r.brow * ALLOC_CHUNK;
-    const double t = tp[r.c];
+    const double den = 2.2204e-16 + *total, t = tp[r.c];
     double pv[MINE];
 #pragma unroll
     for (int m = 0; m < MINE; ++m) { const uint32_t i = (uint32_t)((wv + WAVES * m) * WAVE) + lane; pv[m] = i < r.n ? v[i] : 0.0; }
 #pragma unroll
     for (int m = 0; m < MINE; ++m) {
         const uint32_t k = wv + WAVES * m, i = k * WAVE + lane;
-        double s = i < r.n ? pv[m] / t : 0.0;
+        double s = i < r.n ? (pv[m] / den) / t : 0.0;
 #pragma unroll
         for (int d = 1; d < WAVE; d <<= 1) { const double u = shfl_up_f64(s, d); if ((int)lane >= d) s = s + u; }
         pv[m] = s;
@@ -309,9 +338,8 @@
 void launch_alloc_bgather(hipStream_t s, const double* w, const AllocPlan& pl, const double* gathered, double* brow, int* bmap) {
     if (pl.n_boundary) hipLaunchKernelGGL(k_alloc_bgather, dim3(pl.n_boundary), dim3(256), 0, s, w, pl, gathered, brow, bmap);
 }
-void launch_alloc_chunk_sum(hipStream_t s, const double* w, const double* brow, const AllocPlan& pl, double* part) {
-    const uint32_t nq = pl.n_interior + pl.n_boundary;
-    if (nq) hipLaunchKernelGGL(k_alloc_chunk_sum, dim3(cdiv(nq, 4)), dim3(256), 0, s, w, brow, pl, part);
+void launch_alloc_chunk_sum(hipStream_t s, const double* brow, const AllocPlan& pl, double* part) {
+    if (pl.n_boundary) hipLaunchKernelGGL(k_alloc_chunk_sum, dim3(cdiv(pl.n_boundary, 4)), dim3(256), 0, s, brow, pl, part);
 }
 void launch_tree_sum(hipStream_t s, const double* part, uint32_t nch, double* scratch, double* total) {
     if (nch == 0) { (void)hipMemsetAsync(total, 0, 8, s); return; }
@@ -324,7 +352,7 @@
         cur = dst; nxt += ng; n = ng;
     }
 }
-void launch_alloc_norm(hipStream_t s, double* w, double* brow, const int* bmap, const AllocPlan& pl, const double* total, unsigned long long reads,
+void launch_alloc_norm(hipStream_t s, const double* w, const double* brow, const int* bmap, const AllocPlan& pl, const double* total, unsigned long long reads,
                        uint32_t* rn, double* tp, uint32_t* crn, unsigned long long* sum_rn) {
     const uint32_t nq = pl.n_interior + pl.n_boundary;
     if (nq) hipLaunchKernelGGL(k_alloc_norm, dim3(cdiv(nq, 4)), dim3(256), 0, s, w, brow, bmap, pl, total, reads, rn, tp, crn);
@@ -346,9 +374,9 @@
     scan_all_dev(s, tp, nch, probs, scratch);
     hipLaunchKernelGGL(k_alloc_top_draws, dim3(cdiv((uint64_t)nch + 1024, 256)), dim3(256), 0, s, probs, nch, reads, sum_rn, sum_quota, key, quota);
 }
-void launch_alloc_sample(hipStream_t s, const double* w, const double* brow, const int* bmap, const AllocPlan& pl, const double* tp, const uint32_t* quota, RngKey key, uint32_t* rn) {
+void launch_alloc_sample(hipStream_t s, const double* w, const double* brow, const int* bmap, const AllocPlan& pl, const double* total, const double* tp, const uint32_t* quota, RngKey key, uint32_t* rn) {
     const uint32_t nq = pl.n_interior + pl.n_boundary;
-    if (nq) hipLaunchKernelGGL(k_alloc_sample, dim3(nq), dim3(256), 0, s, w, brow, bmap, pl, tp, quota, key, rn);
+    if (nq) hipLaunchKernelGGL(k_alloc_sample, dim3(nq), dim3(256), 0, s, w, brow, bmap, pl, total, tp, quota, key, rn);
 }
 void launch_alloc_odd_scan(hipStream_t s, const uint32_t* rn, uint32_t ac, uint32_t* odd_before, void* temp, size_t temp_bytes) {
     (void)rocprim::exclusive_scan(temp, temp_bytes, rocprim::make_transform_iterator(rn, OddBit()), odd_before, 0u, (size_t)ac + 1, rocprim::plus<uint32_t>(), s);
@@ -359,9 +387,9 @@
 void launch_alloc_parity(hipStream_t s, uint32_t* rn, const uint32_t* odd_before, uint32_t ac, const AllocPlan& pl, const unsigned long long* table) {
     if (ac) hipLaunchKernelGGL(k_alloc_parity, dim3(cdiv(ac, 256)), dim3(256), 0, s, rn, odd_before, ac, pl, table);
 }
-void launch_weights(hipStream_t s, DevAmps fulls, uint32_t n, DevTables tb, RngKey key, uint32_t frag_size, double* w) {
-    if (n == 0) return;
-    hipLaunchKernelGGL(k_weights, dim3(cdiv(n, (uint32_t)WEIGHTS_BLOCK)), dim3(WEIGHTS_BLOCK), 0, s, fulls, n, tb, key, frag_size, w);
+void launch_weights(hipStream_t s, DevAmps fulls, const AllocPlan& pl, DevTables tb, RngKey key, uint32_t frag_size, double* w, double* part) {
+    const uint32_t nw = pl.n_interior + pl.n_gap;
+    if (nw) hipLaunchKernelGGL(k_weights, dim3(cdiv(nw, (uint32_t)WEIGHTS_WAVES)), dim3(WEIGHTS_WAVES * WAVE), 0, s, fulls, pl, tb, key, frag_size, w, part);
 }
 using ScanCfg = rocprim::scan_config<256, 16, rocprim::block_load_method::block_load_transpose, rocprim::block_store_method::block_store_transpose, rocprim::block_scan_algorithm::using_warp_scan>;
 struct PackOddHalf { __host__ __device__ uint64_t operator()(uint32_t v) const { return ((uint64_t)(v & 1u) << 32) | (uint64_t)(v >> 1); } };
diff --git a/scssim_amd/csrc/scs_reads.cpp b/scssim_amd/csrc/scs_reads.cpp
--- a/scssim_amd/csrc/scs_reads.cpp
+++ b/scssim_amd/csrc/scs_reads.cpp
@@ -17,7 +17,6 @@
     double t0 = now_s();
     c->weights.reserve(std::max<size_t>((size_t)ac * 8, 16), s);
     c->read_numbers.reserve(((size_t)ac + 1) * 4, s); c->pair_off.reserve(((size_t)ac + 1) * 4, s);
-    launch_weights(s, c->fulls.view(), ac, c->dtb, c->key, (uint32_t)c->cfg.frag_size, c->weights.as<double>());
     double* d_w = c->weights.as<double>(); uint32_t* d_rn = c->read_numbers.as<uint32_t>();
 
     const int R = c->cfg.shard_count, me = c->cfg.shard_rank; const bool multi = c->sharded();
@@ -36,10 +35,11 @@
     if (loff[me] != ac) throw ScsError(SCS_EINVAL, "sharded allocation: segment bookkeeping mismatch");
     if (total > 0xFFFFFFF0ull) throw ScsError(SCS_EOVERFLOW, "more than 2^32 amplicons in the whole job");
     const uint32_t nch = (uint32_t)((total + ALLOC_CHUNK - 1) / ALLOC_CHUNK);
-    std::vector<AllocRange> rng; std::vector<AllocBChunk> bch; uint32_t nq = 0;
+    std::vector<AllocRange> rng; std::vector<AllocBChunk> bch; std::vector<AllocGap> gap; uint32_t nq = 0;
     {
         auto owner_of = [&](uint64_t gi) { size_t lo = 0, hi = gseg.size(); while (hi - lo > 1) { const size_t mid = (lo + hi) / 2; if (gseg[mid].go <= gi) lo = mid; else hi = mid; } return gseg[lo].owner; };
         auto add_boundary = [&](uint32_t ch) { for (auto& b : bch) if (b.c == ch) return; bch.push_back(AllocBChunk{ch, (uint32_t)std::min<uint64_t>(ALLOC_CHUNK, total - (uint64_t)ch * ALLOC_CHUNK), owner_of((uint64_t)ch * ALLOC_CHUNK) == (uint32_t)me ? 1u : 0u}); };
+        auto add_gap = [&](uint64_t lo, uint64_t n) { for (; n; lo += std::min<uint64_t>(n, ALLOC_CHUNK), n -= std::min<uint64_t>(n, ALLOC_CHUNK)) gap.push_back(AllocGap{(uint32_t)lo, (uint32_t)std::min<uint64_t>(n, ALLOC_CHUNK)}); };
         for (size_t k = 0; k < gseg.size();) {
             if (gseg[k].owner != (uint32_t)me) { ++k; continue; }
             uint64_t go = gseg[k].go, n = gseg[k].n; const uint32_t lo = gseg[k].lo; size_t j = k + 1;
@@ -47,24 +47,25 @@
             k = j;
             const uint64_t cA = (go + ALLOC_CHUNK - 1) / ALLOC_CHUNK, cB = go + n == total ? nch : (go + n) / ALLOC_CHUNK;
             if (cA < cB) { rng.push_back(AllocRange{nq, (uint32_t)cA, (uint32_t)(lo + (cA * ALLOC_CHUNK - go))}); nq += (uint32_t)(cB - cA); }
-            if (cA >= cB) { for (uint64_t ch = go / ALLOC_CHUNK; ch <= (go + n - 1) / ALLOC_CHUNK; ++ch) add_boundary((uint32_t)ch); }
+            if (cA >= cB) { for (uint64_t ch = go / ALLOC_CHUNK; ch <= (go + n - 1) / ALLOC_CHUNK; ++ch) add_boundary((uint32_t)ch); add_gap(lo, n); }
             else {
-                if (go % ALLOC_CHUNK) add_boundary((uint32_t)(go / ALLOC_CHUNK));
-                if (cB * ALLOC_CHUNK < go + n) add_boundary((uint32_t)cB);
+                if (go % ALLOC_CHUNK) { add_boundary((uint32_t)(go / ALLOC_CHUNK)); add_gap(lo, cA * ALLOC_CHUNK - go); }
+                if (cB * ALLOC_CHUNK < go + n) { add_boundary((uint32_t)cB); add_gap(lo + (cB * ALLOC_CHUNK - go), go + n - cB * ALLOC_CHUNK); }
             }
         }
     }
-    pl.total = total; pl.n_interior = nq; pl.n_boundary = (uint32_t)bch.size(); pl.n_ranges = (uint32_t)rng.size(); pl.n_gseg = (uint32_t)gseg.size();
+    pl.total = total; pl.n_interior = nq; pl.n_boundary = (uint32_t)bch.size(); pl.n_ranges = (uint32_t)rng.size(); pl.n_gseg = (uint32_t)gseg.size(); pl.n_gap = (uint32_t)gap.size();
     const uint32_t nwork = pl.n_interior + pl.n_boundary;
     {
-        const size_t o_b = rng.size() * sizeof(AllocRange), o_g = o_b + bch.size() * sizeof(AllocBChunk), bytes = o_g + gseg.size() * sizeof(AllocGSeg);
+        const size_t o_b = rng.size() * sizeof(AllocRange), o_g = o_b + bch.size() * sizeof(AllocBChunk), o_p = o_g + gseg.size() * sizeof(AllocGSeg), bytes = o_p + gap.size() * sizeof(AllocGap);
         std::vector<uint8_t> blob(std::max<size_t>(bytes, 16));
         if (!rng.empty()) memcpy(blob.data(), rng.data(), o_b);
         if (!bch.empty()) memcpy(blob.data() + o_b, bch.data(), o_g - o_b);
-        if (!gseg.empty()) memcpy(blob.data() + o_g, gseg.data(), bytes - o_g);
+        if (!gseg.empty()) memcpy(blob.data() + o_g, gseg.data(), o_p - o_g);
+        if (!gap.empty()) memcpy(blob.data() + o_p, gap.data(), bytes - o_p);
         c->a_plan.reserve(blob.size(), s);
         HIP_OK(hipMemcpyAsync(c->a_plan.p, blob.data(), blob.size(), hipMemcpyHostToDevice, s)); HIP_OK(hipStreamSynchronize(s));
-        pl.rng = (const AllocRange*)c->a_plan.p; pl.bchunk = (const AllocBChunk*)((char*)c->a_plan.p + o_b); pl.gseg = (const AllocGSeg*)((char*)c->a_plan.p + o_g);
+        pl.rng = (const AllocRange*)c->a_plan.p; pl.bchunk = (const AllocBChunk*)((char*)c->a_plan.p + o_b); pl.gseg = (const AllocGSeg*)((char*)c->a_plan.p + o_g); pl.gap = (const AllocGap*)((char*)c->a_plan.p + o_p);
     }
     for (int sl = 0; sl < ALLOC_SLOTS; ++sl) c->seg_lo[sl] = pl.my_seg[sl].lo;
     c->seg_lo[ALLOC_SLOTS] = ac;
@@ -79,6 +80,8 @@
     AllocState* st = (AllocState*)((char*)c->dsums.p + 128);
     double* d_part = c->a_part.as<double>(); double* d_tp = c->a_tp.as<double>();
     unsigned long long* d_sum_rn = (unsigned long long*)(d_tp + nch);
+    if (multi) HIP_OK(hipMemsetAsync(d_part, 0, (size_t)nch * 8, s));
+    launch_weights(s, c->fulls.view(), pl, c->dtb, c->key, (uint32_t)c->cfg.frag_size, d_w, d_part);
     if (R > 1) {
         const size_t per = (size_t)ALLOC_SLOTS * 2 * ALLOC_CHUNK * 8;
         c->a_send.reserve(per, s); c->a_gath.reserve(per * R, s);
@@ -86,15 +89,14 @@
         c->gather_dev(c->a_send.p, c->a_gath.p, per);
     }
     launch_alloc_bgather(s, d_w, pl, c->a_gath.as<double>(), c->a_brow.as<double>(), c->a_bmap.as<int>());
-    if (multi) HIP_OK(hipMemsetAsync(d_part, 0, (size_t)nch * 8, s));
-    launch_alloc_chunk_sum(s, d_w, c->a_brow.as<double>(), pl, d_part);
+    launch_alloc_chunk_sum(s, c->a_brow.as<double>(), pl, d_part);
     if (multi) c->reduce_dev(d_part, nch, 8);
     launch_tree_sum(s, d_part, nch, c->a_scratch.as<double>(), &st->total);
     if (multi) HIP_OK(hipMemsetAsync(d_tp, 0, ((size_t)nch + 1) * 8, s));
     launch_alloc_norm(s, d_w, c->a_brow.as<double>(), c->a_bmap.as<int>(), pl, &st->total, reads, d_rn, d_tp, c->a_crn.as<uint32_t>(), d_sum_rn);
     if (multi) c->reduce_dev(d_tp, (uint64_t)nch + 1, 8);
     launch_alloc_quota(s, d_tp, nch, reads, d_sum_rn, &st->sum_quota, c->a_quota.as<uint32_t>(), c->a_probs.as<double>(), c->a_scratch.as<double>(), c->key);
-    launch_alloc_sample(s, d_w, c->a_brow.as<double>(), c->a_bmap.as<int>(), pl, d_tp, c->a_quota.as<uint32_t>(), c->key, d_rn);
+    launch_alloc_sample(s, d_w, c->a_brow.as<double>(), c->a_bmap.as<int>(), pl, &st->total, d_tp, c->a_quota.as<uint32_t>(), c->key, d_rn);
     if (c->cfg.paired && !multi) launch_parity_pair_offsets(s, d_rn, ac, c->pair_off.as<uint32_t>(), c->scan_tmp.p, c->scan_tmp.cap);
     else if (c->cfg.paired) {
         launch_alloc_odd_scan(s, d_rn, ac, c->odd_before.as<uint32_t>(), c->scan_tmp.p, c->scan_tmp.cap);
```

New measurement: 52.93 million. 0.968x the previous value.
